# yaomy533/pose_estimation

Hardware: AMD Instinct MI355X
Metric: crops/sec at 640×480 RGB-D, 1000 sampled pts; ADD(-S) AUC vs reference (higher is better)
Workload: dtype f32; 1 GPU; LineMOD 'cat' batch=64/GPU, 120x120 crops from 640x480 RGB-D, HRNet-W18 + 1000-pt fusion + TBase, PnP-RANSAC (H=100) on GPU; batch_per_gpu=64, global_batch=64, crop=120, points=1000, backbone=hrnet_w18, parallelism=single, graph=True, micro_batches=1, pipeline=none, graph_branches=True

## Files before the change

include/krrn_hip.h:

```cpp
#ifndef KRRN_HIP_H
#define KRRN_HIP_H

#include <stdint.h>

#ifdef __cplusplus
extern "C" {
#endif

#define KRRN_OK 0
#define KRRN_EARG (-1)
#define KRRN_ESHAPE (-2)
#define KRRN_EALIGN (-3)
#define KRRN_EUNSUPPORTED (-4)

int krrn_conv2d_f32(const float* in, int in_cs, int in_co, int B, int Hi, int Wi, int cin, int Hg, int Wg,
                    int in_s, int ntaps, const int* tap_dy, const int* tap_dx, const float* wt, int N,
                    int n_store, const float* scale, const float* bias, const float* bias2, int b2_div,
                    const float* res, int res_cs, int res_co, float* out, int out_cs, int out_co, int Ho,
                    int Wo, int osy, int osx, int ooy, int oox, int relu, int out_nchw, int tile, int splits,
                    float* workspace, void* stream);

typedef struct krrn_conv_desc {
  const float* in;
  int in_cs, in_co, B, Hi, Wi, cin, Hg, Wg, in_s, ntaps;
  int tap_dy[9];
  int tap_dx[9];
  const float* wt;
  int N, n_store;
  const float* scale;
  const float* bias;
  const float* bias2;
  int b2_div;
  const float* res;
  int res_cs, res_co;
  float* out;
  int out_cs, out_co, Ho, Wo, osy, osx, ooy, oox, relu, out_nchw, splits;
  float* workspace;
  int k_chunk;
} krrn_conv_desc;

int krrn_conv2d_group_f32(const krrn_conv_desc* descs, int n, int tile, void* stream);

int krrn_conv2d_x3_f32(const float* in, int in_cs, int in_co, int B, int Hi, int Wi, int cin, int Hg, int Wg,
                       int in_s, int ntaps, const int* tap_dy, const int* tap_dx, const void* wt3, int N, int n_store,
                       const float* scale, const float* bias, const float* bias2, int b2_div, const float* res,
                       int res_cs, int res_co, float* out, int out_cs, int out_co, int Ho, int Wo, int osy, int osx,
                       int ooy, int oox, int relu, int tile, int splits, float* workspace, void* stream);
int krrn_conv2d_group_x3_f32(const krrn_conv_desc* descs, int n, int tile, void* stream);
int krrn_convT_s2_x3_f32(const float* in, int in_cs, int in_co, int B, int Hi, int Wi, int cin, const int* cls_taps,
                         const void* U3, int N, const float* scale, const float* bias, int relu, float* out,
                         int out_cs, int out_co, int Ho, int Wo, void* stream);

typedef struct krrn_blas_gemm krrn_blas_gemm;
int krrn_blas_gemm_create(int M, int N, int K, int lda, int ldo, int batch, long long a_grp, long long o_grp,
                          int has_bias, int relu, int has_res, int ldr, long long r_grp, long long max_ws,
                          krrn_blas_gemm** out_plan, long long* ws_bytes);
int krrn_blas_gemm_run(const krrn_blas_gemm* g, const float* a, const float* w, const float* bias, const float* res,
                       float* out, void* workspace, long long ws_bytes, void* stream);
int krrn_blas_gemm_destroy(krrn_blas_gemm* g);

int krrn_gemm_x3_f32(const float* a, int lda, int M, int K, int N, const void* w3f, const float* bias,
                     const float* res, int ldr, float* out, int ldo, int relu, int batch, long long a_grp,
                     long long o_grp, long long r_grp, void* stream);

int krrn_gemm_x3_gather_f32(const int* ia, const float* A, long long a_bs, int a_st, const int* ib, const float* A2,
                            long long a2_bs, int a2_st, int npts, int B, int K, int N, const void* w3f,
                            const float* bias, float* out, int ldo, int relu, void* stream);

int krrn_gemm_panel_x3_f32(const float* a, int lda, int M, int K, int N, const void* wpf, const float* bias,
                           const float* res, int ldr, float* out, int ldo, int relu, int csplit, void* stream);

int krrn_conv1x1_nchw_f32(const float* in, int in_cs, int in_co, int B, int HW, int cin, const float* wt, int N,
                          int n_store, const float* scale, const float* bias, float* out, int out_cs, int out_co,
                          void* stream);

int krrn_conv1x1_nchw_x3_f32(const float* in, int in_cs, int in_co, int B, int HW, int cin, const void* w3, int N,
                             int n_store, const float* scale, const float* bias, float* out, int out_cs, int out_co,
                             void* stream);

int krrn_conv3x3_wino_f32(const float* in, int in_cs, int in_co, int B, int H, int W, int cin, const float* U,
                          int N, int n_store, const float* scale, const float* bias, const float* res, int res_cs,
                          int res_co, float* out, int out_cs, int out_co, int relu, void* stream);
int krrn_conv3x3_wino_x3_f32(const float* in, int in_cs, int in_co, int B, int H, int W, int cin, const void* U3,
                             int N, int n_store, const float* scale, const float* bias, const float* res, int res_cs,
                             int res_co, float* out, int out_cs, int out_co, int relu, void* stream);
int krrn_conv3x3_wino4_x3_f32(const float* in, int in_cs, int in_co, int B, int H, int W, int cin, const void* U3,
                              int N, int n_store, const float* scale, const float* bias, const float* res, int res_cs,
                              int res_co, float* out, int out_cs, int out_co, int relu, void* stream);
int krrn_conv3x3_wino4_x3_head_f32(const float* in, int in_cs, int in_co, int B, int H, int W, int cin,
                                   const void* U3, int N, const float* scale, const float* bias, const float* res,
                                   int res_cs, int res_co, int relu, const float* w1, const float* b1, int p1,
                                   float* part, float* out, int out_c, void* stream);
int krrn_conv3x3_wino_x3_head_f32(const float* in, int in_cs, int in_co, int B, int H, int W, int cin,
                                  const void* U3, int N, const float* scale, const float* bias, const float* res,
                                  int res_cs, int res_co, int relu, const float* w1, const float* b1, int p1,
                                  float* part, float* out, int out_c, void* stream);

int krrn_conv_small_f32(const float* in, int in_cs, int in_co, int B, int H, int W, int cin, const float* wt, int N,
                        int n_store, const float* scale, const float* bias, const float* res, int res_cs, int res_co,
                        float* out, int out_cs, int out_co, int relu, int ksize, int stride, int nw, int ks,
                        void* stream);


int krrn_knn_f32(const float* q, long long q_bs, int q_st, int nq, const int* qidx, const float* c,
                 long long c_bs, int c_st, int nc, int d, int k, int drop_first, int mode, int B, int* out,
                 void* stream);

int krrn_gcn_conv_f32(const int* idx, int n, int k, const float* v, long long v_bs, int v_st, int d,
                      const float* dn, int S, int C, const float* Y, const float* bn_scale, const float* bn_bias,
                      int relu, float* out, long long o_bs, int o_st, int B, void* stream);

int krrn_pool_max_f32(const int* nbr, int nq, int kk, const float* F, long long f_bs, int f_st, int C, float* out,
                      long long o_bs, int o_st, int B, void* stream);

int krrn_resize_bilinear_f32(const float* in, int B, int Hi, int Wi, int in_cs, int in_co, int C, float* out,
                             int Ho, int Wo, int out_cs, int out_co, const float* add, int add_cs, int add_co,
                             int align_corners, int relu, void* stream);

int krrn_add_relu_f32(const float* a, int a_cs, int a_co, const float* b, int b_cs, int b_co, float* out,
                      int o_cs, int o_co, long long npix, int C, int relu, void* stream);

int krrn_nchw_to_nhwc_f32(const float* in, int B, int C, int H, int W, float* out, int o_cs, int o_co,
                          void* stream);

int krrn_heads_select_f32(const float* fx, int Cx, int xyz_off, const float* fn, int Cn, const long long* cls,
                          float* xyz_out, float* nml_out, int B, int H, int W, void* stream);

int krrn_points_gather_f32(const float* cloud, const float* xyz, const float* nml, const long long* choose, int B,
                           int N, int H, int W, float* p9, void* stream);

int krrn_gather_rows_f32(const void* idx, int idx64, long long idx_bs, int nrows, const float* src, long long src_bs,
                         int src_st, float* dst, long long dst_bs, int dst_st, int width, int B, void* stream);

int krrn_gather2_add_f32(const int* ia, const float* A, long long a_bs, int a_st, const int* ib, const float* B_,
                         long long b_bs, int b_st, int n, int C, const float* scale, const float* bias,
                         const float* bias2, int relu, float* out, long long o_bs, int o_st, int B, void* stream);

int krrn_tbase_tail_f32(const float* h, int B, int n, int C, const float* w4, const float* b4, const float* cloud,
                        float* pred_t, float* t_res, void* stream);

int krrn_pnp_ransac_f32(const float* xyz, int HW, const long long* choose, int N, const int* sel, int P,
                        const float* xmap, const float* ymap, const float* K4, const double* extent,
                        const double* lfborder, const int* subsets, int H, float thr, double conf, float* workspace,
                        float* R, float* t, int* inliers, unsigned char* inlier_mask, int B, void* stream);

int krrn_model_points_f32(const float* xyz, int HW, const long long* choose, int N, const double* extent,
                          const double* lfborder, float* out, int B, void* stream);

int krrn_umeyama_ransac_f32(const float* src, const float* dst, int N, const int* subsets, int H,
                            double inlier_frac, double conf, double min_ratio, int* hyp_counts,
                            float* scale, float* R, float* t, int* inliers, int* best_hyp,
                            unsigned char* inlier_mask, int B, void* stream);

int krrn_icp_refine_f32(const float* R0, const float* t0, const float* cloud, int N, const float* model, int M,
                        const float* max_dist, int max_iter, double tol, int min_pairs, float* R, float* t,
                        int* passes, int* pairs, float* rmse, int* status, int* nn_idx, int B, void* stream);

int krrn_randperm_i32(const unsigned long long* seed_ptr, unsigned int stream_id, int n, int k, int rows, int* out,
                      void* stream);

int krrn_randperm_multi_i32(const unsigned long long* seed_ptr, int count, const unsigned int* stream_id, const int* n,
                            const int* k, int* const* out, void* stream);

int krrn_ransac_subsets(const unsigned long long* seed_ptr, unsigned int stream_id, int B, int H, int P, int* out,
                        void* stream);

int krrn_rng_advance(unsigned long long* seed_ptr, void* stream);

int krrn_map_losses_ws(int B, int HW, long long* n_doubles);
int krrn_map_losses_f32(const float* xyz, const float* xyz_gt, const float* nml, const float* nml_gt,
                        const float* region, int R, const long long* region_gt, const float* mask, int M,
                        const long long* mask_gt, int B, int HW, double* ws, double* out, void* stream);
int krrn_map_losses_crop_f32(const double* ws, int B, int HW, double* out_crop, void* stream);

int krrn_pose_loss_ws(int B, int P, long long* n_doubles);
int krrn_pose_loss_f32(const float* target_r, const float* pred_t, const float* target, const float* model_points,
                       const long long* cls_id, const int* sym, int nsym, int B, int P, double* ws, double* out,
                       void* stream);

int krrn_add_metric_f32(const float* pred_r, const float* pred_t, const float* model_points, const float* target,
                        const long long* cls_id, const int* sym, int nsym, int B, int P, double* ws, double* out,
                        void* stream);

int krrn_crop_inputs_u8(const unsigned char* rgb, const float* depth, const unsigned char* mask_label,
                        const unsigned char* obj_mask, int F, int H, int W, const int* frame, const int* rc, int B,
                        int S, float* img, unsigned char* mask, void* stream);

int krrn_choose_points(const unsigned char* mask, int B, int S, int N, const float* depth, int H, int W,
                       const int* frame, const int* rc, const float* K4, float depth_scale, const long long* seed,
                       int stream_id, long long* choose, float* cloud, float* xmap, float* ymap, int* count,
                       void* stream);

int krrn_fps_f32(const float* pts, int B, int n, int n_samples, int* out_idx, void* stream);

int krrn_raster_maps_f32(const float* verts, int Vtot, const int* faces, int Ftot, const int* face_range,
                         const double* R, const double* t, const float* K4, const int* rc, int S,
                         const float* region_pts, int NR, int B, int* face, float* depth, float* coord,
                         float* normal, int* region, unsigned char* cover_frame, int H, int W, void* stream);

int krrn_gt_maps_finish_f32(const float* coord, const int* region_raw, const int* face,
                            const unsigned char* point_mask, const long long* cls, const double* extent,
                            const double* lfborder, int B, int HW, float* xyz, float* normal, long long* region,
                            float* mask, long long* multi_cls_mask, float* mask_obj, void* stream);

int krrn_bop_vsd_ws(int B, long long* n_ints);
int krrn_bop_vsd_f32(const float* verts, int Vtot, const int* faces, int Ftot, const int* face_range,
                     const double* R_est, const double* t_est, const double* R_gt, const double* t_gt,
                     const float* K4, const float* depth, int F, int H, int W, const int* frame, double depth_scale,
                     const double* diameter, double delta, const double* taus, int T, int B, int* ws, int* counts,
                     double* e_vsd, void* stream);

int krrn_bop_visib_ws(int B, long long* n_ints);
int krrn_bop_visib_u8(const float* verts, int Vtot, const int* faces, int Ftot, const int* face_range,
                      const double* R, const double* t, const float* K4, const float* depth, int F, int H, int W,
                      const int* frame, double depth_scale, double delta, int B, int* ws,
                      unsigned char* mask, unsigned char* mask_visib, int* info, double* visib_fract,
                      void* stream);

int krrn_bop_mssd_mspd_ws(int B, long long* n_doubles);
int krrn_bop_mssd_mspd_f32(const float* verts, int Vtot, const int* vert_range, const double* R_est,
                           const double* t_est, const double* R_gt, const double* t_gt, const float* K4,
                           const double* syms, int NStot, const int* sym_range, int B, double* ws, double* mssd,
                           double* mspd, int* sym_idx, void* stream);

int krrn_bpnp_solve_f32(const float* pts2d, const float* pts3d, int z_per_crop, const float* K, const float* y_init,
                        const float* R_init, int B, int n, int iters, float* y_out, float* cost_out, void* stream);

int krrn_bpnp_backward_f32(const float* pts2d, const float* P6, const float* pts3d, int z_per_crop, const float* K,
                           const float* grad_out, int B, int n, float* grad_x, float* grad_z, float* grad_K,
                           double* workspace, void* stream);

#ifdef __cplusplus
}
#endif

#endif
```

pose_estimation_amd/csrc/gemm_x3.hip:

```cpp
#include "krrn_common.h"
#include "krrn_split.h"

namespace {

constexpr int BM = 128, BN = 128;
constexpr int KC = 16;
constexpr int NG = KC / 8;
constexpr int PX = 3 * KC + 4;

struct GemmArgs {
  const float* a;
  const float* a2;
  const int* ia;
  const int* ib;
  long long a2_grp;
  int lda2, npts;
  const unsigned* w;
  const float* bias;
  const float* res;
  float* out;
  int lda, M, K, N, ldr, ldo, relu;
  long long a_grp, o_grp, r_grp;
  int mt, nt, total;
};

__device__ __forceinline__ void split_quads(const f32x4 x, u32x4& q0, u32x4& q1, u32x4& q2) {
  const KrrnSplit3 s = krrn_split3(x);
  q0 = u32x4{s.h0, s.h1, s.h0, s.h1};
  q1 = u32x4{s.h0, s.h1, s.m0, s.m1};
  q2 = u32x4{s.m0, s.m1, s.l0, s.l1};
}

template <bool GA>
__global__ __launch_bounds__(256, 2) void gemm_x3_kernel(const GemmArgs g) {
  __shared__ __attribute__((aligned(16))) unsigned smem[2 * BM * PX];

  const int tpg = g.mt * g.nt;
  const int bid = krrn_xcd_remap(blockIdx.x, g.total);
  const int grp = bid / tpg, rem = bid - grp * tpg;
  const int tm = rem / g.nt, tn = rem - tm * g.nt;
  const int m0 = tm * BM, n0 = tn * BN;
  const int tid = threadIdx.x, lane = tid & 63, wave = tid >> 6;
  const int frow = lane & 31, fh = lane >> 5;

  const int srow = tid >> 2, kq = (tid & 3) * 4;
  const float* abase = GA ? g.a : g.a + grp * g.a_grp + (size_t)m0 * g.lda;
  const int rows = min(BM, g.M - m0);
  const __amdgpu_buffer_rsrc_t rsA = __builtin_amdgcn_make_buffer_rsrc(
      (void*)abase, (short)0, GA ? (int)(g.a_grp * (g.M / g.npts) * 4) : ((rows - 1) * g.lda + g.K) * 4, 0x00020000);
  __amdgpu_buffer_rsrc_t rsA2;
  unsigned aoff[2], aoff2[2];
  if constexpr (GA) {
    rsA2 = __builtin_amdgcn_make_buffer_rsrc((void*)g.a2, (short)0, (int)(g.a2_grp * (g.M / g.npts) * 4),
                                             0x00020000);
#pragma unroll
    for (int i = 0; i < 2; ++i) {
      const int m = m0 + srow + 64 * i;
      if (m < g.M) {
        const int b = m / g.npts;
        aoff[i] = (unsigned)((b * g.a_grp + (long long)g.ia[m] * g.lda + kq) * 4);
        aoff2[i] = (unsigned)((b * g.a2_grp + (long long)g.ib[m] * g.lda2 + kq) * 4);
      } else {
        aoff[i] = aoff2[i] = 0x80000000u;
      }
    }
  } else {
#pragma unroll
    for (int i = 0; i < 2; ++i) aoff[i] = (unsigned)(((srow + 64 * i) * g.lda + kq) * 4);
  }

  const int G = g.K >> 3;
  const unsigned* wb = g.w + ((size_t)((n0 >> 5) + wave) * G) * 512 + lane * 4;

  const int nch = g.K / KC;
  f32x4 ra[2][2];
  f32x4 rq[GA ? 2 : 1][2];
  auto load_a = [&](int c, int s) {
    c = min(c, nch - 1);
#pragma unroll
    for (int i = 0; i < 2; ++i) {
      ra[s][i] = __builtin_bit_cast(
          f32x4, __builtin_amdgcn_raw_buffer_load_b128(rsA, aoff[i] + (unsigned)(c * KC * 4), 0, 0));
      if constexpr (GA)
        rq[s][i] = __builtin_bit_cast(
            f32x4, __builtin_amdgcn_raw_buffer_load_b128(rsA2, aoff2[i] + (unsigned)(c * KC * 4), 0, 0));
    }
  };
  auto store_a = [&](int s) {
    unsigned* d = smem + s * BM * PX;
#pragma unroll
    for (int i = 0; i < 2; ++i) {
      u32x4 q0, q1, q2;
      f32x4 x = ra[s][i];
      if constexpr (GA) {
        x += rq[s][i];
#pragma unroll
        for (int e = 0; e < 4; ++e) x[e] = fmaxf(x[e], 0.f);
      }
      split_quads(x, q0, q1, q2);
      unsigned* p = d + (srow + 64 * i) * PX + 3 * kq;
      *reinterpret_cast<u32x4*>(p) = q0;
      *reinterpret_cast<u32x4*>(p + 4) = q1;
      *reinterpret_cast<u32x4*>(p + 8) = q2;
    }
  };
  u32x4 wr[4][2];
  auto load_w = [&](int gi, int s) {
    const unsigned* p = wb + (size_t)min(gi, G - 1) * 512;
    wr[s][0] = *reinterpret_cast<const u32x4*>(p);
    wr[s][1] = *reinterpret_cast<const u32x4*>(p + 256);
  };

  f32x16 acc[4];
#pragma unroll
  for (int i = 0; i < 4; ++i)
#pragma unroll
    for (int r = 0; r < 16; ++r) acc[i][r] = 0.f;
  typedef u32x4 Frag[4][3];
  auto read_frag = [&](int buf, int gl, Frag& f) {
    const unsigned* As = smem + buf * BM * PX;
#pragma unroll
    for (int i = 0; i < 4; ++i) {
      const unsigned* p = As + (i * 32 + frow) * PX + 12 * (2 * gl + fh);
#pragma unroll
      for (int q = 0; q < 3; ++q) f[i][q] = *reinterpret_cast<const u32x4*>(p + 4 * q);
    }
  };
  auto mma = [&](const Frag& f, int s) {
    const bf16x8 p0 = krrn_op(wr[s][0]), p1 = krrn_op(wr[s][1]);
#pragma unroll
    for (int i = 0; i < 4; ++i) {
      acc[i] = __builtin_amdgcn_mfma_f32_32x32x16_bf16(krrn_op(f[i][0]), p0, acc[i], 0, 0, 0);
      acc[i] = __builtin_amdgcn_mfma_f32_32x32x16_bf16(krrn_op(f[i][1]), p1, acc[i], 0, 0, 0);
      acc[i] = __builtin_amdgcn_mfma_f32_32x32x16_bf16(krrn_op(f[i][2]), p1, acc[i], 0, 0, 0);
    }
  };

  static_assert(NG == 2, "the chunk schedule below is written for 2 groups per chunk");
  Frag fa, fb;
  load_a(0, 0);
  load_a(1, 1);
  load_w(0, 0);
  load_w(1, 1);
  store_a(0);
  __syncthreads();
  load_a(2, 0);
  read_frag(0, 0, fa);
  for (int c = 0; c < nch; c += 2) {
#pragma unroll
    for (int h = 0; h < 2; ++h) {
      const int gi = (c + h) * NG;
      __builtin_amdgcn_sched_barrier(0);
      load_w(gi + 2, (2 * h + 2) & 3);
      read_frag(h, 1, fb);
      store_a(1 - h);
      mma(fa, 2 * h);
      __builtin_amdgcn_sched_group_barrier(0x020, 2, 0);
      __builtin_amdgcn_sched_group_barrier(0x100, 12, 0);
#pragma unroll
      for (int q = 0; q < 12; ++q) {
        __builtin_amdgcn_sched_group_barrier(0x008, 1, 0);
        __builtin_amdgcn_sched_group_barrier(0x002, 6, 0);
        if (q < 6) __builtin_amdgcn_sched_group_barrier(0x200, 1, 0);
      }
      __builtin_amdgcn_sched_barrier(0);
      __syncthreads();
      load_a(c + h + 3, 1 - h);
      load_w(gi + 3, (2 * h + 3) & 3);
      read_frag(1 - h, 0, fa);
      __builtin_amdgcn_sched_barrier(0);
      mma(fb, 2 * h + 1);
    }
  }
  __builtin_amdgcn_sched_barrier(0);

  __syncthreads();
  constexpr int TP = 36;
  float* const ts = reinterpret_cast<float*>(smem) + wave * (32 * TP);
  const int trow = lane >> 3, tcol = 4 * (lane & 7);
  const int nq = n0 + wave * 32 + tcol;
  float bq[4];
#pragma unroll
  for (int e = 0; e < 4; ++e) bq[e] = g.bias ? g.bias[nq + e] : 0.f;
  float* ob = g.out + grp * g.o_grp + nq;
  const float* rb = g.res ? g.res + grp * g.r_grp + nq : nullptr;
#pragma unroll
  for (int i = 0; i < 4; ++i) {
#pragma unroll
    for (int r = 0; r < 16; ++r) ts[((r & 3) + 8 * (r >> 2) + 4 * fh) * TP + frow] = acc[i][r];
    __builtin_amdgcn_wave_barrier();
    f32x4 tv[4];
#pragma unroll
    for (int j = 0; j < 4; ++j) tv[j] = *reinterpret_cast<const f32x4*>(ts + (8 * j + trow) * TP + tcol);
    __builtin_amdgcn_wave_barrier();
#pragma unroll
    for (int j = 0; j < 4; ++j) {
      const int m = m0 + i * 32 + 8 * j + trow;
      if (m >= g.M) continue;
      f32x4 v = tv[j];
#pragma unroll
      for (int e = 0; e < 4; ++e) {
        v[e] += bq[e];
        if (rb) v[e] += rb[(size_t)m * g.ldr + e];
        if (g.relu) v[e] = fmaxf(v[e], 0.f);
      }
      *reinterpret_cast<f32x4*>(ob + (size_t)m * g.ldo) = v;
    }
  }
}

}

KRRN_API int krrn_gemm_x3_f32(const float* a, int lda, int M, int K, int N, const void* w3f, const float* bias,
                              const float* res, int ldr, float* out, int ldo, int relu, int batch, long long a_grp,
                              long long o_grp, long long r_grp, void* stream) {
  if (!a || !w3f || !out) return KRRN_EARG;
  if (M < 1 || K < KC || N < BN || batch < 1) return KRRN_ESHAPE;
  if ((K % (2 * KC)) || (N % BN) || lda < K || ldo < N) return KRRN_ESHAPE;
  if ((lda & 3) || (ldo & 3) || (a_grp & 3) || (o_grp & 3)) return KRRN_EALIGN;
  if (res && ((ldr != 0 && ldr < N) || (r_grp & 3))) return KRRN_ESHAPE;
  if (!krrn_aligned16(a) || !krrn_aligned16(w3f) || !krrn_aligned16(out)) return KRRN_EALIGN;
  if ((long long)BM * lda * 4 >= 0x7FFFFFFFLL) return KRRN_ESHAPE;
  const long long tiles = (long long)krrn_cdiv(M, BM) * (N / BN) * batch;
  if (tiles > 0x7FFFFFFFLL) return KRRN_ESHAPE;
  GemmArgs g;
  g.a = a; g.a2 = nullptr; g.ia = g.ib = nullptr; g.a2_grp = 0; g.lda2 = 0; g.npts = 1;
  g.w = reinterpret_cast<const unsigned*>(w3f); g.bias = bias; g.res = res; g.out = out;
  g.lda = lda; g.M = M; g.K = K; g.N = N; g.ldr = ldr; g.ldo = ldo; g.relu = relu;
  g.a_grp = a_grp; g.o_grp = o_grp; g.r_grp = r_grp;
  g.mt = krrn_cdiv(M, BM); g.nt = N / BN; g.total = (int)tiles;
  hipLaunchKernelGGL(gemm_x3_kernel<false>, dim3((unsigned)tiles), dim3(256), 0, (hipStream_t)stream, g);
  return krrn_launch_status();
}

KRRN_API int krrn_gemm_x3_gather_f32(const int* ia, const float* A, long long a_bs, int a_st, const int* ib,
                                     const float* A2, long long a2_bs, int a2_st, int npts, int B, int K, int N,
                                     const void* w3f, const float* bias, float* out, int ldo, int relu,
                                     void* stream) {
  if (!ia || !A || !ib || !A2 || !w3f || !out) return KRRN_EARG;
  if (npts < 1 || B < 1 || K < KC || N < BN) return KRRN_ESHAPE;
  if ((K % (2 * KC)) || (N % BN) || a_st < K || a2_st < K || ldo < N) return KRRN_ESHAPE;
  if ((a_st & 3) || (a2_st & 3) || (a_bs & 3) || (a2_bs & 3) || (ldo & 3)) return KRRN_EALIGN;
  if (!krrn_aligned16(A) || !krrn_aligned16(A2) || !krrn_aligned16(w3f) || !krrn_aligned16(out)) return KRRN_EALIGN;
  if ((long long)B * a_bs * 4 >= 0x7FFFFFFFLL || (long long)B * a2_bs * 4 >= 0x7FFFFFFFLL) return KRRN_ESHAPE;
  const long long M = (long long)B * npts;
  const long long tiles = (long long)krrn_cdiv(M, BM) * (N / BN);
  if (M > 0x7FFFFFFFLL || tiles > 0x7FFFFFFFLL) return KRRN_ESHAPE;
  GemmArgs g;
  g.a = A; g.a2 = A2; g.ia = ia; g.ib = ib; g.a_grp = a_bs; g.a2_grp = a2_bs; g.lda = a_st; g.lda2 = a2_st;
  g.npts = npts;
  g.w = reinterpret_cast<const unsigned*>(w3f); g.bias = bias; g.res = nullptr; g.out = out;
  g.M = (int)M; g.K = K; g.N = N; g.ldr = 0; g.ldo = ldo; g.relu = relu;
  g.o_grp = 0; g.r_grp = 0;
  g.mt = krrn_cdiv(g.M, BM); g.nt = N / BN; g.total = (int)tiles;
  hipLaunchKernelGGL(gemm_x3_kernel<true>, dim3((unsigned)tiles), dim3(256), 0, (hipStream_t)stream, g);
  return krrn_launch_status();
}
```

pose_estimation_amd/csrc/pointwise.hip:

```cpp
#include <math.h>

#include "krrn_common.h"

namespace {

template <typename IT>
__global__ void resize_bilinear_kernel(const float* __restrict__ in, int Hi, int Wi, int in_cs, int in_co, int C4,
                                       float* __restrict__ out, int Ho, int Wo, int out_cs, int out_co,
                                       const float* __restrict__ add, int add_cs, int add_co, float sh, float sw,
                                       int align, int relu, IT total) {
  const IT e = (IT)blockIdx.x * blockDim.x + threadIdx.x;
  if (e >= total) return;
  const int c4 = (int)(e % C4);
  IT p = e / C4;
  const int ox = (int)(p % Wo);
  p /= Wo;
  const int oy = (int)(p % Ho);
  const int b = (int)(p / Ho);
  int y0, y1, x0, x1;
  float ly0, ly1, lx0, lx1;
  krrn_src_index(oy, Hi, sh, align, y0, y1, ly0, ly1);
  krrn_src_index(ox, Wi, sw, align, x0, x1, lx0, lx1);
  const float* ib = in + (long long)b * Hi * Wi * in_cs + in_co + 4 * c4;
  const f32x4 v00 = *reinterpret_cast<const f32x4*>(ib + ((long long)y0 * Wi + x0) * in_cs);
  const f32x4 v01 = *reinterpret_cast<const f32x4*>(ib + ((long long)y0 * Wi + x1) * in_cs);
  const f32x4 v10 = *reinterpret_cast<const f32x4*>(ib + ((long long)y1 * Wi + x0) * in_cs);
  const f32x4 v11 = *reinterpret_cast<const f32x4*>(ib + ((long long)y1 * Wi + x1) * in_cs);
  f32x4 r = krrn_bilerp4(v00, v01, v10, v11, ly0, ly1, lx0, lx1);
  const long long opix = ((long long)b * Ho + oy) * Wo + ox;
  if (add) r = *reinterpret_cast<const f32x4*>(add + opix * add_cs + add_co + 4 * c4) + r;
  if (relu) {
    r.x = fmaxf(r.x, 0.f); r.y = fmaxf(r.y, 0.f); r.z = fmaxf(r.z, 0.f); r.w = fmaxf(r.w, 0.f);
  }
  *reinterpret_cast<f32x4*>(out + opix * out_cs + out_co + 4 * c4) = r;
}

__device__ __forceinline__ f32x4 pick3(const f32x4 (&r)[3], int i) { return i == 0 ? r[0] : (i == 1 ? r[1] : r[2]); }

__global__ void resize_up2x2_kernel(const float* __restrict__ in, int Hi, int Wi, int in_cs, int in_co, int C4,
                                    float* __restrict__ out, int Ho, int Wo, int out_cs, int out_co,
                                    const float* __restrict__ add, int add_cs, int add_co, float sh, float sw,
                                    int align, int relu, int Ho2, int Wo2, int total) {
  const int e = blockIdx.x * blockDim.x + threadIdx.x;
  if (e >= total) return;
  const int c4 = e % C4;
  int p = e / C4;
  const int ox2 = p % Wo2;
  p /= Wo2;
  const int oy2 = p % Ho2;
  const int b = p / Ho2;
  int y0[2], y1[2], x0[2], x1[2];
  float ly0[2], ly1[2], lx0[2], lx1[2];
#pragma unroll
  for (int d = 0; d < 2; ++d) {
    krrn_src_index(min(2 * oy2 + d, Ho - 1), Hi, sh, align, y0[d], y1[d], ly0[d], ly1[d]);
    krrn_src_index(min(2 * ox2 + d, Wo - 1), Wi, sw, align, x0[d], x1[d], lx0[d], lx1[d]);
  }
  const float* ib = in + (long long)b * Hi * Wi * in_cs + in_co + 4 * c4;
  f32x4 P[3][3];
#pragma unroll
  for (int r = 0; r < 3; ++r)
#pragma unroll
    for (int c = 0; c < 3; ++c) {
      const int yy = min(y0[0] + r, Hi - 1), xx = min(x0[0] + c, Wi - 1);
      P[r][c] = *reinterpret_cast<const f32x4*>(ib + ((long long)yy * Wi + xx) * in_cs);
    }
#pragma unroll
  for (int dy = 0; dy < 2; ++dy) {
    const int oy = 2 * oy2 + dy;
    if (oy >= Ho) break;
    const int ra = y0[dy] - y0[0], rb = y1[dy] - y0[0];
    f32x4 row0[3], row1[3];
#pragma unroll
    for (int c = 0; c < 3; ++c) {
      row0[c] = ra == 0 ? P[0][c] : P[1][c];
      row1[c] = rb == 0 ? P[0][c] : (rb == 1 ? P[1][c] : P[2][c]);
    }
#pragma unroll
    for (int dx = 0; dx < 2; ++dx) {
      const int ox = 2 * ox2 + dx;
      if (ox >= Wo) break;
      const int ca = x0[dx] - x0[0], cb = x1[dx] - x0[0];
      const f32x4 v00 = pick3(row0, ca), v01 = pick3(row0, cb), v10 = pick3(row1, ca), v11 = pick3(row1, cb);
      f32x4 r = krrn_bilerp4(v00, v01, v10, v11, ly0[dy], ly1[dy], lx0[dx], lx1[dx]);
      const long long opix = ((long long)b * Ho + oy) * Wo + ox;
      if (add) r = *reinterpret_cast<const f32x4*>(add + opix * add_cs + add_co + 4 * c4) + r;
      if (relu) {
        r.x = fmaxf(r.x, 0.f); r.y = fmaxf(r.y, 0.f); r.z = fmaxf(r.z, 0.f); r.w = fmaxf(r.w, 0.f);
      }
      *reinterpret_cast<f32x4*>(out + opix * out_cs + out_co + 4 * c4) = r;
    }
  }
}

template <typename IT>
__global__ void add_relu_kernel(const float* __restrict__ a, int a_cs, int a_co, const float* __restrict__ b,
                                int b_cs, int b_co, float* __restrict__ out, int o_cs, int o_co, int C4, int relu,
                                IT total) {
  const IT e = (IT)blockIdx.x * blockDim.x + threadIdx.x;
  if (e >= total) return;
  const int c4 = (int)(e % C4);
  const long long pix = e / C4;
  f32x4 r = *reinterpret_cast<const f32x4*>(a + pix * a_cs + a_co + 4 * c4);
  if (b) r = r + *reinterpret_cast<const f32x4*>(b + pix * b_cs + b_co + 4 * c4);
  if (relu) {
    r.x = fmaxf(r.x, 0.f); r.y = fmaxf(r.y, 0.f); r.z = fmaxf(r.z, 0.f); r.w = fmaxf(r.w, 0.f);
  }
  *reinterpret_cast<f32x4*>(out + pix * o_cs + o_co + 4 * c4) = r;
}

__global__ void nchw_to_nhwc_kernel(const float* __restrict__ in, int C, int HW, float* __restrict__ out, int o_cs,
                                    int o_co, long long total) {
  const long long e = (long long)blockIdx.x * blockDim.x + threadIdx.x;
  if (e >= total) return;
  const int p = (int)(e % HW);
  const long long bc = e / HW;
  const int c = (int)(bc % C);
  const long long b = bc / C;
  out[(b * HW + p) * o_cs + o_co + c] = in[e];
}

__global__ void heads_select_kernel(const float* __restrict__ fx, int Cx, int xyz_off, const float* __restrict__ fn,
                                    int Cn, const long long* __restrict__ cls, float* __restrict__ xyz,
                                    float* __restrict__ nml, int HW, long long total) {
  const long long e = (long long)blockIdx.x * blockDim.x + threadIdx.x;
  if (e >= total) return;
  const int p = (int)(e % HW);
  const long long b = e / HW;
  const int c = (int)cls[b];
  const float* sx = fx + (b * Cx + xyz_off + 3 * c) * HW + p;
  const float* sn = fn + (b * Cn + 3 * c) * HW + p;
  float* dx = xyz + b * 3 * HW + p;
  float* dn = nml + b * 3 * HW + p;
  dx[0] = sx[0];
  dx[HW] = sx[HW];
  dx[2 * HW] = sx[2 * HW];
  const float n0 = sn[0], n1 = sn[HW], n2 = sn[2 * HW];
  const float nr = fmaxf(sqrtf(n0 * n0 + n1 * n1 + n2 * n2), 1e-12f);
  dn[0] = n0 / nr;
  dn[HW] = n1 / nr;
  dn[2 * HW] = n2 / nr;
}

__global__ void points_gather_kernel(const float* __restrict__ cloud, const float* __restrict__ xyz,
                                     const float* __restrict__ nml, const long long* __restrict__ choose, int N,
                                     int HW, float* __restrict__ p9, long long total) {
  const long long e = (long long)blockIdx.x * blockDim.x + threadIdx.x;
  if (e >= total) return;
  const long long b = e / N;
  const long long pix = choose[e];
  float* o = p9 + e * 9;
  const float* cl = cloud + e * 3;
  o[0] = cl[0];
  o[1] = cl[1];
  o[2] = cl[2];
  const float* x = xyz + b * 3 * HW + pix;
  const float* n = nml + b * 3 * HW + pix;
  o[3] = x[0];
  o[4] = x[HW];
  o[5] = x[2 * HW];
  o[6] = n[0];
  o[7] = n[HW];
  o[8] = n[2 * HW];
}

template <bool IDX64, bool VEC>
__global__ void gather_rows_kernel(const void* __restrict__ idx, long long idx_bs, int nrows,
                                   const float* __restrict__ src, long long src_bs, int src_st,
                                   float* __restrict__ dst, long long dst_bs, int dst_st, int width,
                                   long long total) {
  const long long e = (long long)blockIdx.x * blockDim.x + threadIdx.x;
  if (e >= total) return;
  const int wq = VEC ? width / 4 : width;
  const int w = (int)(e % wq);
  const long long br = e / wq;
  const int r = (int)(br % nrows);
  const long long b = br / nrows;
  const long long ii = b * idx_bs + r;
  const long long row = IDX64 ? ((const long long*)idx)[ii] : (long long)((const int*)idx)[ii];
  const float* s = src + b * src_bs + row * src_st;
  float* d = dst + b * dst_bs + (long long)r * dst_st;
  if constexpr (VEC) {
    *reinterpret_cast<f32x4*>(d + 4 * w) = *reinterpret_cast<const f32x4*>(s + 4 * w);
  } else {
    d[w] = s[w];
  }
}

constexpr int kTailWaves = 16;
__global__ __launch_bounds__(64 * kTailWaves) void tbase_tail_kernel(const float* __restrict__ h, int n, int C,
                                                         const float* __restrict__ w4,
                                                         const float* __restrict__ b4,
                                                         const float* __restrict__ cloud,
                                                         float* __restrict__ pred_t, float* __restrict__ t_res) {
  __shared__ float red[kTailWaves][3];
  const int b = blockIdx.x;
  const int lane = threadIdx.x & 63, wave = threadIdx.x >> 6;
  const int q = lane & 3, pl = lane >> 2;
  const int C4 = C >> 2;
  const float bx = b4[0], by = b4[1], bz = b4[2];
  float sx = 0.f, sy = 0.f, sz = 0.f;
  for (int i0 = 0; i0 < n; i0 += 16 * kTailWaves) {
    const int i = i0 + wave * 16 + pl;
    if (i < n) {
      const f32x4* hr = reinterpret_cast<const f32x4*>(h + ((long long)b * n + i) * C);
      float a0 = 0.f, a1 = 0.f, a2 = 0.f;
      for (int c4 = q; c4 < C4; c4 += 4) {
        const f32x4 x = hr[c4];
        const f32x4 w0 = reinterpret_cast<const f32x4*>(w4)[c4];
        const f32x4 w1 = reinterpret_cast<const f32x4*>(w4 + C)[c4];
        const f32x4 w2 = reinterpret_cast<const f32x4*>(w4 + 2 * C)[c4];
        a0 += w0[0] * x[0] + w0[1] * x[1] + w0[2] * x[2] + w0[3] * x[3];
        a1 += w1[0] * x[0] + w1[1] * x[1] + w1[2] * x[2] + w1[3] * x[3];
        a2 += w2[0] * x[0] + w2[1] * x[1] + w2[2] * x[2] + w2[3] * x[3];
      }
      a0 += __shfl_xor(a0, 1);
      a1 += __shfl_xor(a1, 1);
      a2 += __shfl_xor(a2, 1);
      a0 += __shfl_xor(a0, 2);
      a1 += __shfl_xor(a1, 2);
      a2 += __shfl_xor(a2, 2);
      if (q == 0) {
        const float t0 = a0 + bx, t1 = a1 + by, t2 = a2 + bz;
        if (t_res) {
          float* tr = t_res + ((long long)b * n + i) * 3;
          tr[0] = t0; tr[1] = t1; tr[2] = t2;
        }
        const float* cp = cloud + ((long long)b * n + i) * 3;
        sx += cp[0] + t0;
        sy += cp[1] + t1;
        sz += cp[2] + t2;
      }
    }
  }
#pragma unroll
  for (int off = 4; off < 64; off <<= 1) {
    sx += __shfl_xor(sx, off);
    sy += __shfl_xor(sy, off);
    sz += __shfl_xor(sz, off);
  }
  if (lane == 0) {
    red[wave][0] = sx; red[wave][1] = sy; red[wave][2] = sz;
  }
  __syncthreads();
  if (threadIdx.x < 3) {
    const int j = threadIdx.x;
    float acc = 0.f;
#pragma unroll
    for (int w = 0; w < kTailWaves; ++w) acc += red[w][j];
    pred_t[b * 3 + j] = acc / (float)n;
  }
}

template <typename IT>
__global__ void gather2_add_kernel(const int* __restrict__ ia, const float* __restrict__ A, long long a_bs, int a_st,
                                   const int* __restrict__ ib, const float* __restrict__ Bm, long long b_bs,
                                   int b_st, int n, int C4, const float* __restrict__ scale,
                                   const float* __restrict__ bias, const float* __restrict__ bias2, int relu,
                                   float* __restrict__ out, long long o_bs, int o_st, IT total) {
  const IT e = (IT)blockIdx.x * blockDim.x + threadIdx.x;
  if (e >= total) return;
  const int c4 = (int)(e % C4);
  const IT bi = e / C4;
  const int i = (int)(bi % n);
  const int b = (int)(bi / n);
  const int ra = ia[(long long)b * n + i], rb = ib[(long long)b * n + i];
  const f32x4 x = *reinterpret_cast<const f32x4*>(A + b * a_bs + (long long)ra * a_st + 4 * c4) +
                  *reinterpret_cast<const f32x4*>(Bm + b * b_bs + (long long)rb * b_st + 4 * c4);
  f32x4 v = x * *reinterpret_cast<const f32x4*>(scale + 4 * c4) + *reinterpret_cast<const f32x4*>(bias + 4 * c4);
  if (bias2) v += *reinterpret_cast<const f32x4*>(bias2 + (long long)b * 4 * C4 + 4 * c4);
  if (relu) {
    v.x = fmaxf(v.x, 0.f); v.y = fmaxf(v.y, 0.f); v.z = fmaxf(v.z, 0.f); v.w = fmaxf(v.w, 0.f);
  }
  *reinterpret_cast<f32x4*>(out + b * o_bs + (long long)i * o_st + 4 * c4) = v;
}

inline dim3 grid1(long long total) { return dim3((unsigned)((total + 255) / 256)); }

}

KRRN_API int krrn_resize_bilinear_f32(const float* in, int B, int Hi, int Wi, int in_cs, int in_co, int C,
                                      float* out, int Ho, int Wo, int out_cs, int out_co, const float* add,
                                      int add_cs, int add_co, int align_corners, int relu, void* stream) {
  if (!in || !out) return KRRN_EARG;
  if (B < 1 || Hi < 1 || Wi < 1 || Ho < 1 || Wo < 1 || C < 1) return KRRN_ESHAPE;
  if ((C & 3) || (in_cs & 3) || (in_co & 3) || (out_cs & 3) || (out_co & 3) || !krrn_aligned16(in) ||
      !krrn_aligned16(out))
    return KRRN_EALIGN;
  if (add && ((add_cs & 3) || (add_co & 3) || !krrn_aligned16(add))) return KRRN_EALIGN;
  float sh, sw;
  if (align_corners) {
    sh = Ho > 1 ? (float)(Hi - 1) / (float)(Ho - 1) : 0.f;
    sw = Wo > 1 ? (float)(Wi - 1) / (float)(Wo - 1) : 0.f;
  } else {
    sh = (float)Hi / (float)Ho;
    sw = (float)Wi / (float)Wo;
  }
  const int Ho2 = (Ho + 1) / 2, Wo2 = (Wo + 1) / 2;
  const long long total2 = (long long)B * Ho2 * Wo2 * (C / 4);
  constexpr long long up_min = 1LL << 21;
  if (Ho >= Hi && Wo >= Wi && total2 >= up_min && total2 < 0x7fffffffLL) {
    hipLaunchKernelGGL(resize_up2x2_kernel, grid1(total2), dim3(256), 0, (hipStream_t)stream, in, Hi, Wi, in_cs, in_co,
                       C / 4, out, Ho, Wo, out_cs, out_co, add, add_cs, add_co, sh, sw, align_corners, relu, Ho2, Wo2,
                       (int)total2);
    return krrn_launch_status();
  }
  const long long total = (long long)B * Ho * Wo * (C / 4);
  if (total < 0x7fffffffLL)
    hipLaunchKernelGGL(resize_bilinear_kernel<int>, grid1(total), dim3(256), 0, (hipStream_t)stream, in, Hi, Wi,
                       in_cs, in_co, C / 4, out, Ho, Wo, out_cs, out_co, add, add_cs, add_co, sh, sw, align_corners,
                       relu, (int)total);
  else
    hipLaunchKernelGGL(resize_bilinear_kernel<long long>, grid1(total), dim3(256), 0, (hipStream_t)stream, in, Hi,
                       Wi, in_cs, in_co, C / 4, out, Ho, Wo, out_cs, out_co, add, add_cs, add_co, sh, sw,
                       align_corners, relu, total);
  return krrn_launch_status();
}

KRRN_API int krrn_add_relu_f32(const float* a, int a_cs, int a_co, const float* b, int b_cs, int b_co, float* out,
                               int o_cs, int o_co, long long npix, int C, int relu, void* stream) {
  if (!a || !out) return KRRN_EARG;
  if (npix < 1 || C < 1) return KRRN_ESHAPE;
  if ((C & 3) || (a_cs & 3) || (a_co & 3) || (o_cs & 3) || (o_co & 3) || (b && ((b_cs & 3) || (b_co & 3))))
    return KRRN_EALIGN;
  if (!krrn_aligned16(a) || !krrn_aligned16(out) || (b && !krrn_aligned16(b))) return KRRN_EALIGN;
  const long long total = npix * (C / 4);
  if (total < 0x7fffffffLL)
    hipLaunchKernelGGL(add_relu_kernel<int>, grid1(total), dim3(256), 0, (hipStream_t)stream, a, a_cs, a_co, b, b_cs,
                       b_co, out, o_cs, o_co, C / 4, relu, (int)total);
  else
    hipLaunchKernelGGL(add_relu_kernel<long long>, grid1(total), dim3(256), 0, (hipStream_t)stream, a, a_cs, a_co, b,
                       b_cs, b_co, out, o_cs, o_co, C / 4, relu, total);
  return krrn_launch_status();
}

KRRN_API int krrn_nchw_to_nhwc_f32(const float* in, int B, int C, int H, int W, float* out, int o_cs, int o_co,
                                   void* stream) {
  if (!in || !out) return KRRN_EARG;
  if (B < 1 || C < 1 || H < 1 || W < 1 || o_co + C > o_cs) return KRRN_ESHAPE;
  const long long total = (long long)B * C * H * W;
  hipLaunchKernelGGL(nchw_to_nhwc_kernel, grid1(total), dim3(256), 0, (hipStream_t)stream, in, C, H * W, out, o_cs,
                     o_co, total);
  return krrn_launch_status();
}

KRRN_API int krrn_heads_select_f32(const float* fx, int Cx, int xyz_off, const float* fn, int Cn,
                                   const long long* cls, float* xyz_out, float* nml_out, int B, int H, int W,
                                   void* stream) {
  if (!fx || !fn || !cls || !xyz_out || !nml_out) return KRRN_EARG;
  if (B < 1 || H < 1 || W < 1 || Cx < xyz_off + 3 || Cn < 3) return KRRN_ESHAPE;
  const long long total = (long long)B * H * W;
  hipLaunchKernelGGL(heads_select_kernel, grid1(total), dim3(256), 0, (hipStream_t)stream, fx, Cx, xyz_off, fn, Cn,
                     cls, xyz_out, nml_out, H * W, total);
  return krrn_launch_status();
}

KRRN_API int krrn_points_gather_f32(const float* cloud, const float* xyz, const float* nml, const long long* choose,
                                    int B, int N, int H, int W, float* p9, void* stream) {
  if (!cloud || !xyz || !nml || !choose || !p9) return KRRN_EARG;
  if (B < 1 || N < 1 || H < 1 || W < 1) return KRRN_ESHAPE;
  const long long total = (long long)B * N;
  hipLaunchKernelGGL(points_gather_kernel, grid1(total), dim3(256), 0, (hipStream_t)stream, cloud, xyz, nml, choose,
                     N, H * W, p9, total);
  return krrn_launch_status();
}

KRRN_API int krrn_gather_rows_f32(const void* idx, int idx64, long long idx_bs, int nrows, const float* src,
                                  long long src_bs, int src_st, float* dst, long long dst_bs, int dst_st, int width,
                                  int B, void* stream) {
  if (!idx || !src || !dst) return KRRN_EARG;
  if (B < 1 || nrows < 1 || width < 1) return KRRN_ESHAPE;
  const bool vec = !(width & 3) && !(src_st & 3) && !(dst_st & 3) && !(src_bs & 3) && !(dst_bs & 3) &&
                   krrn_aligned16(src) && krrn_aligned16(dst);
  const long long total = (long long)B * nrows * (vec ? width / 4 : width);
  hipStream_t s = (hipStream_t)stream;
#define KRRN_GR(I64, V)                                                                                    \
  hipLaunchKernelGGL((gather_rows_kernel<I64, V>), grid1(total), dim3(256), 0, s, idx, idx_bs, nrows, src, \
                     src_bs, src_st, dst, dst_bs, dst_st, width, total)
  if (idx64) {
    if (vec) KRRN_GR(true, true); else KRRN_GR(true, false);
  } else {
    if (vec) KRRN_GR(false, true); else KRRN_GR(false, false);
  }
#undef KRRN_GR
  return krrn_launch_status();
}

KRRN_API int krrn_tbase_tail_f32(const float* h, int B, int n, int C, const float* w4, const float* b4,
                                 const float* cloud, float* pred_t, float* t_res, void* stream) {
  if (!h || !w4 || !b4 || !cloud || !pred_t) return KRRN_EARG;
  if (B < 1 || n < 1 || C < 1) return KRRN_ESHAPE;
  if ((C & 3) || !krrn_aligned16(h) || !krrn_aligned16(w4)) return KRRN_EALIGN;
  hipLaunchKernelGGL(tbase_tail_kernel, dim3(B), dim3(64 * kTailWaves), 0, (hipStream_t)stream, h, n, C, w4, b4, cloud, pred_t,
                     t_res);
  return krrn_launch_status();
}

KRRN_API int krrn_gather2_add_f32(const int* ia, const float* A, long long a_bs, int a_st, const int* ib, const float* B_,
                                  long long b_bs, int b_st, int n, int C, const float* scale, const float* bias,
                                  const float* bias2, int relu, float* out, long long o_bs, int o_st, int B,
                                  void* stream) {
  if (!ia || !A || !ib || !B_ || !scale || !bias || !out) return KRRN_EARG;
  if (n < 1 || C < 1 || B < 1) return KRRN_ESHAPE;
  if ((C & 3) || (a_st & 3) || (b_st & 3) || (o_st & 3) || (a_bs & 3) || (b_bs & 3) || (o_bs & 3) ||
      !krrn_aligned16(A) || !krrn_aligned16(B_) || !krrn_aligned16(out) || !krrn_aligned16(scale) ||
      !krrn_aligned16(bias) || (bias2 && !krrn_aligned16(bias2)))
    return KRRN_EALIGN;
  const long long total = (long long)B * n * (C / 4);
  if (total < 0x7fffffffLL)
    hipLaunchKernelGGL(gather2_add_kernel<int>, grid1(total), dim3(256), 0, (hipStream_t)stream, ia, A, a_bs, a_st, ib,
                       B_, b_bs, b_st, n, C / 4, scale, bias, bias2, relu, out, o_bs, o_st, (int)total);
  else
    hipLaunchKernelGGL(gather2_add_kernel<long long>, grid1(total), dim3(256), 0, (hipStream_t)stream, ia, A, a_bs,
                       a_st, ib, B_, b_bs, b_st, n, C / 4, scale, bias, bias2, relu, out, o_bs, o_st, total);
  return krrn_launch_status();
}
```

pose_estimation_amd/fusion.py:

```python
from __future__ import annotations

import math
from typing import Callable, Dict, List, Optional

import torch
import torch.nn as nn
import torch.nn.functional as F

from . import knobs, ops
from .runtime import Late, Plan, add_conv, add_gemm, ptr


class Conv_surface(nn.Module):
    def __init__(self, kernel_num, support_num):
        super().__init__()
        self.kernel_num = kernel_num
        self.support_num = support_num
        self.directions = nn.Parameter(torch.empty(3, support_num * kernel_num))
        stdv = 1.0 / math.sqrt(support_num * kernel_num)
        nn.init.uniform_(self.directions, -stdv, stdv)


class Conv_layer(nn.Module):
    dim = 3

    def __init__(self, in_channel, out_channel, support_num):
        super().__init__()
        self.in_channel, self.out_channel, self.support_num = in_channel, out_channel, support_num
        self.weights = nn.Parameter(torch.empty(in_channel, (support_num + 1) * out_channel))
        self.bias = nn.Parameter(torch.empty((support_num + 1) * out_channel))
        self.directions = nn.Parameter(torch.empty(self.dim, support_num * out_channel))
        stdv = 1.0 / math.sqrt(out_channel * (support_num + 1))
        for p in (self.weights, self.bias, self.directions):
            nn.init.uniform_(p, -stdv, stdv)


class Conv_fuse_layer(Conv_layer):
    dim = 9


class Pool_layer(nn.Module):
    def __init__(self, pooling_rate: int = 4, neighbor_num: int = 4):
        super().__init__()
        self.pooling_rate = pooling_rate
        self.neighbor_num = neighbor_num


class FusionNetLite(nn.Module):
    def __init__(self, cfg):
        super().__init__()
        self.neighbor_num = cfg.Module.GCN3D.GCN_N_NUM
        self.support_num = cfg.Module.GCN3D.GCN_SUP_NUM
        self.num_cls = cfg.Module.NUM_CLS
        S = self.support_num
        for br in ("v", "x", "n"):
            setattr(self, f"conv_0_{br}", Conv_surface(128, S))
            setattr(self, f"conv_1_{br}", Conv_layer(128, 128, S))
            setattr(self, f"pool_1_{br}", Pool_layer(4, 4))
            setattr(self, f"conv_2_{br}", Conv_layer(128, 128, S))
            setattr(self, f"bn1_{br}", nn.BatchNorm1d(128))
            setattr(self, f"bn2_{br}", nn.BatchNorm1d(128))
        self.pool_1 = Pool_layer(4, 4)
        self.pool_2 = Pool_layer(4, 4)
        self.conv_4 = Conv_fuse_layer(384, 512, S)
        self.conv_5 = Conv_fuse_layer(512, 512, S)



FEAT_SID = 4
FUSION_CHUNK = knobs.integer("KRRN_FUSION_CHUNK")

def level_sizes(N: int, k0: int):
    N1 = int(N / 4)
    N2 = int(N1 / 4)
    k1 = min(k0, N1 // 8)
    k2 = min(k0, N2 // 8)
    return N1, N2, k1, k2


def _dn(directions: torch.Tensor, device) -> torch.Tensor:
    return F.normalize(directions.detach().float().cpu(), dim=0).contiguous().to(device)


def _bn1d(bn: nn.BatchNorm1d, device):
    s = (bn.weight.detach().double() / torch.sqrt(bn.running_var.detach().double() + bn.eps))
    b = bn.bias.detach().double() - bn.running_mean.detach().double() * s
    return s.float().to(device), b.float().to(device)


class _Emit:

    def __init__(self, fu: FusionNetLite, plan: Plan, B: int, keep: list):
        self.plan, self.B, self.dev, self.S, self.keep = plan, B, plan.device, fu.support_num, keep
        self._lin: dict = {}

    def knn(self, q, q_bs, q_st, nq, qidx, c, c_bs, c_st, nc, d, k, drop, mode, out):
        self.plan.add("krrn_knn_f32", q, q_bs, q_st, nq, qidx, c, c_bs, c_st, nc, d, k, drop, mode, self.B, ptr(out))

    def gcn(self, idx, n, k, v, v_bs, d, dn, C, Y, bn, relu, out, o_bs, o_st, Bc=None, v_st=9):
        self.keep.append(dn)
        s, b = (None, None) if bn is None else bn
        self.keep.extend([s, b])
        self.plan.add("krrn_gcn_conv_f32", ptr(idx), n, k, v, v_bs, v_st, d, ptr(dn), self.S, C, ptr(Y), ptr(s), ptr(b),
                      int(relu), out, o_bs, o_st, self.B if Bc is None else Bc)

    def gemm(self, a, a_cs, a_co, M, layer: "Conv_layer", out):
        spec = self._lin.get(id(layer))
        if spec is None:
            spec = ops.make_linear(layer.weights.detach().t(), layer.bias, None, self.dev,
                                   cin_p=ops.pad4(layer.in_channel))
            self._lin[id(layer)] = spec
            self.keep.append(spec)
        np_ = ops.pad4(spec.cout)
        if add_gemm(self.plan, a=a, a_off=a_co, lda=a_cs, M=M, wt=spec.wt[0], K=spec.cin_p, N=np_, scale=spec.scale,
                    bias=spec.bias, out=out, ldo=out.shape[-1], relu=False, cin=spec.cin, cout=spec.cout,
                    tag="gcn_gemm"):
            return
        add_conv(self.plan, x=ptr(a), x_cs=a_cs, x_co=a_co, B=1, Hi=1, Wi=M, cin_p=spec.cin_p, Hg=1, Wg=M, in_s=1,
                 taps=[(0, 0)], wt=ptr(spec.wt[0]), N=np_, n_store=np_, scale=ptr(spec.scale), bias=ptr(spec.bias),
                 out=ptr(out), out_cs=out.shape[-1], out_co=0, Ho=1, Wo=M, cin=spec.cin, cout=spec.cout,
                 tag="gcn_gemm")


def _off(t, floats):
    return ptr(t) if floats == 0 else type(ptr(t))(t.data_ptr() + 4 * floats)


def _level0_branch(e: _Emit, fu: FusionNetLite, bi: int, br: str, N: int, idx0, v, v_bs, v_st, F0, Y1b, feat1, cy: int):
    B = e.B
    c0 = getattr(fu, f"conv_0_{br}")
    e.gcn(idx0, N, fu.neighbor_num, v, v_bs, 3, _dn(c0.directions, e.dev), 128, None, None, True,
          _off(F0, 128 * bi), N * 384, 384, v_st=v_st)
    c1 = getattr(fu, f"conv_1_{br}")
    dn1, bn1 = _dn(c1.directions, e.dev), _bn1d(getattr(fu, f"bn1_{br}"), e.dev)
    for b0 in range(0, B, cy):
        nb = min(cy, B - b0)
        e.gemm(F0[b0:b0 + nb], 384, 128 * bi, nb * N, c1, Y1b)
        vb = type(v)(v.value + 4 * b0 * v_bs)
        e.gcn(idx0[b0:b0 + nb], N, fu.neighbor_num, vb, v_bs, 3, dn1, 128, Y1b, bn1, True,
              _off(feat1[b0:], 128 * bi), N * 384, 384, Bc=nb, v_st=v_st)


def emit_fusion_cloud_part(fu: FusionNetLite, plan: Plan, B: int, N: int, cloud: torch.Tensor) -> dict:
    k0 = fu.neighbor_num
    keep: list = []
    e = _Emit(fu, plan, B, keep)
    cy = B if not FUSION_CHUNK or FUSION_CHUNK >= B else FUSION_CHUNK
    idx0 = plan.buf((B, N, k0), torch.int32)
    F0 = plan.buf((B, N, 384))
    feat1 = plan.buf((B, N, 384))
    Y1v = plan.buf((cy * N, (fu.support_num + 1) * 128))
    e.knn(ptr(cloud), N * 3, 3, N, ptr(None), ptr(cloud), N * 3, 3, N, 3, k0, 1, 0, idx0)
    _level0_branch(e, fu, 0, "v", N, idx0, ptr(cloud), N * 3, 3, F0, Y1v, feat1, cy)
    plan.buffers.append(keep)
    return dict(idx0=idx0, F0=F0, feat1=feat1, Y1v=Y1v)


def build_fusion_plan(fu: FusionNetLite, plan: Plan, B: int, N: int, p9: torch.Tensor, perms: Dict[str, torch.Tensor],
                      hooks: Optional[Dict[str, List[Callable[[dict], None]]]] = None, materialize: bool = True,
                      early: Optional[dict] = None):
    hooks = hooks or {}
    dev = plan.device
    S = fu.support_num
    k0 = fu.neighbor_num
    N1, N2, k1, k2 = level_sizes(N, k0)
    if k1 < 1 or k2 < 1:
        raise ValueError(f"num_points={N} too small for the 3-level GCN (needs N/16 >= 8)")
    keep = []
    i32 = torch.int32
    idx0 = early["idx0"] if early else plan.buf((B, N, k0), i32)
    F0 = early["F0"] if early else plan.buf((B, N, 384))
    cy = B if not FUSION_CHUNK or FUSION_CHUNK >= B else FUSION_CHUNK
    Y1 = [early["Y1v"] if early and i == 0 else plan.buf((cy * N, (S + 1) * 128)) for i in range(3)]
    feat1 = early["feat1"] if early else plan.buf((B, N, 384))
    nb4 = {br: plan.buf((B, N1, 4), i32) for br in ("v", "x", "n")}
    V1 = plan.buf((B, N1, 9))
    FP1 = plan.buf((B, N1, 384))
    PV1 = plan.buf((B, N1, 9))
    idx1 = plan.buf((B, N1, k1), i32)
    Y2 = [plan.buf((B * N1, (S + 1) * 128)) for _ in range(3)]
    feat2 = plan.buf((B, N1, 384))
    nb4b = plan.buf((B, N2, 4), i32)
    FP2 = plan.buf((B, N2, 384))
    PV2 = plan.buf((B, N2, 9))
    idx2 = plan.buf((B, N2, k2), i32)
    Y4 = plan.buf((B * N2, (S + 1) * 512))
    fm4 = plan.buf((B, N2, 512))
    Y5 = plan.buf((B * N2, (S + 1) * 512))
    fm5 = plan.buf((B, N2, 512))
    nn1 = plan.buf((B, N), i32)
    nn2 = plan.buf((B, N), i32)
    feat = plan.buf((B, N, 1280)) if materialize else None

    e = _Emit(fu, plan, B, keep)
    knn, gcn, gemm, off = e.knn, e.gcn, e.gemm, _off

    if not early:
        knn(off(p9, 0), N * 9, 9, N, ptr(None), off(p9, 0), N * 9, 9, N, 3, k0, 1, 0, idx0)
    plan.fork([1, 2])
    for bi, br in enumerate(("v", "x", "n")):
        with plan.on_stream(bi):
            if not (early and bi == 0):
                _level0_branch(e, fu, bi, br, N, idx0, off(p9, 3 * bi), N * 9, 9, F0, Y1[bi], feat1, cy)
            perm = perms[br]
            knn(off(p9, 3 * bi), N * 9, 9, N1, ptr(perm), off(p9, 3 * bi), N * 9, 9, N, 3, 4, 1, 0, nb4[br])
            plan.add("krrn_pool_max_f32", ptr(nb4[br]), N1, 4, off(feat1, 128 * bi), N * 384, 384, 128,
                     off(FP1, 128 * bi), N1 * 384, 384, B)
            plan.add("krrn_gather_rows_f32", ptr(perm), 0, 0, N1, off(p9, 3 * bi), N * 9, 9, off(V1, 3 * bi),
                     N1 * 9, 9, 3, B)
    plan.add("krrn_gather_rows_f32", ptr(perms["p1"]), 0, 0, N1, off(p9, 0), N * 9, 9, off(PV1, 0), N1 * 9, 9, 9, B)
    plan.join([1, 2])
    knn(off(V1, 0), N1 * 9, 9, N1, ptr(None), off(V1, 0), N1 * 9, 9, N1, 3, k1, 1, 0, idx1)
    plan.fork([1, 2, 3])
    with plan.on_stream(3):
        knn(off(p9, 0), N * 9, 9, N, ptr(None), off(PV1, 0), N1 * 9, 9, N1, 3, 1, 0, 1, nn1)
    for bi, br in enumerate(("v", "x", "n")):
        with plan.on_stream(bi):
            c2 = getattr(fu, f"conv_2_{br}")
            gemm(FP1, 384, 128 * bi, B * N1, c2, Y2[bi])
            gcn(idx1, N1, k1, off(V1, 3 * bi), N1 * 9, 3, _dn(c2.directions, dev), 128, Y2[bi],
                _bn1d(getattr(fu, f"bn2_{br}"), dev), True, off(feat2, 128 * bi), N1 * 384, 384)
    plan.join([1, 2])
    for h in hooks.get("level1", []):
        h(dict(feat1=feat1, feat2=feat2))
    knn(off(PV1, 0), N1 * 9, 9, N2, ptr(perms["p2"]), off(PV1, 0), N1 * 9, 9, N1, 3, 4, 1, 0, nb4b)
    plan.add("krrn_pool_max_f32", ptr(nb4b), N2, 4, off(feat2, 0), N1 * 384, 384, 384, off(FP2, 0), N2 * 384, 384, B)
    plan.add("krrn_gather_rows_f32", ptr(perms["p2"]), 0, 0, N2, off(PV1, 0), N1 * 9, 9, off(PV2, 0), N2 * 9, 9, 9, B)
    knn(off(PV2, 0), N2 * 9, 9, N2, ptr(None), off(PV2, 0), N2 * 9, 9, N2, 9, k2, 1, 0, idx2)
    for h in hooks.get("level2", []):
        h(dict(feat1=feat1, feat2=feat2))
    plan.fork([3])
    with plan.on_stream(3):
        knn(off(p9, 0), N * 9, 9, N, ptr(None), off(PV2, 0), N2 * 9, 9, N2, 3, 1, 0, 1, nn2)
    gemm(FP2, 384, 0, B * N2, fu.conv_4, Y4)
    gcn(idx2, N2, k2, off(PV2, 0), N2 * 9, 9, _dn(fu.conv_4.directions, dev), 512, Y4, None, False,
        off(fm4, 0), N2 * 512, 512)
    gemm(fm4, 512, 0, B * N2, fu.conv_5, Y5)
    gcn(idx2, N2, k2, off(PV2, 0), N2 * 9, 9, _dn(fu.conv_5.directions, dev), 512, Y5, None, False,
        off(fm5, 0), N2 * 512, 512)
    plan.join([3])
    if materialize:
        plan.fork([FEAT_SID])
        with plan.on_stream(FEAT_SID):
            plan.add("krrn_gather_rows_f32", ptr(nn2), 0, N, N, off(fm5, 0), N2 * 512, 512, off(feat, 0), N * 1280,
                     1280, 512, B)
            plan.add("krrn_gather_rows_f32", ptr(nn1), 0, N, N, off(feat1, 0), N * 384, 384, off(feat, 512),
                     N * 1280, 1280, 384, B)
            plan.add("krrn_gather_rows_f32", ptr(nn1), 0, N, N, off(feat2, 0), N1 * 384, 384, off(feat, 896),
                     N * 1280, 1280, 384, B)
    plan.buffers.append(keep)
    return feat, dict(pool_v=nb4["v"], pool_x=nb4["x"], pool_n=nb4["n"], pool2=nb4b, idx0=idx0, idx1=idx1, idx2=idx2, nn1=nn1, nn2=nn2, feat1=feat1, feat2=feat2, fm5=fm5,
                      F0=F0, V1=V1, PV1=PV1, PV2=PV2, FP1=FP1, FP2=FP2, fm4=fm4, Y1=Y1, Y2=Y2, Y4=Y4, Y5=Y5)
```

pose_estimation_amd/knobs.py:

```python
from __future__ import annotations

import os
from typing import Dict, Optional, Tuple

KNOBS: Dict[str, Tuple[Optional[str], str]] = {
    "KRRN_HIP_LIB": (None, "path of the C-ABI library to load instead of the in-tree libkrrn_hip.so "
                           "(variant builds for A/B timing, the KRRN_DIAG diagnostics build)"),
    "KRRN_GRAPH": ("1", "KRRN.forward replays a captured hipGraph of its plan; 0 = serial eager runs"),
    "KRRN_PLAN_STREAMS": ("1", "captured plans keep their side streams as graph branches; 0 = captured serially"),
    "KRRN_STREAMS": ("1", "the two-slot pipeline's stages, concurrent micro-batches and config 3's buckets "
                          "replay side by side on their own streams; 0 = one after the other"),
    "KRRN_PLAN_BUDGET_GB": ("48", "device memory the KRRN plan cache may hold before evicting the least "
                                  "recently used (B, S, N) plan"),
    "KRRN_DIAG_DROP": ("", "comma list of C-ABI entry points left out of new plans: a what-if timing "
                           "diagnostic (profiles/whatif.sh); outputs are meaningless with it set"),
    "KRRN_WINO": ("1", "3x3 stride-1 convs on the Winograd kernels; 0 = the implicit-GEMM conv"),
    "KRRN_WINO_X3": ("1", "Winograd with split-bf16 MFMAs (f32 accuracy); 0 = the f32 Winograd"),
    "KRRN_WINO4": ("1", "the heads' wide 3x3 convs on the split-bf16 Winograd F(4x4, 3x3); 0 = F(2x2, 3x3)"),
    "KRRN_FUSE_EARLY": ("1", "HRNet fuse terms that read one branch start on that branch's stream before the join"),
    "KRRN_MODULE_STREAMS": ("1", "consecutive HRNet modules of a stage keep each branch on its stream (no barrier between them)"),
    "KRRN_STAGE_STREAMS": ("1", "with KRRN_MODULE_STREAMS, HRNet stages chain per branch stream too (transitions on their branch's stream)"),
    "KRRN_FUSION_EARLY": ("1", "the fusion work that reads only the input cloud runs beside the HRNet phase (side stream)"),
    "KRRN_FUSE_EDGES": ("1", "each HRNet fuse output waits for exactly its branches (capture edges); 0 = module barrier"),
    "KRRN_HEAD_FUSE": ("1", "a <= 4-output final 1x1 fused into the head's last split Winograd; 0 = two launches"),
    "KRRN_SMALL_CONV": ("1", "HRNet branch / fuse convs on the LDS-slab conv_small kernel; 0 = implicit GEMM"),
    "KRRN_GEMM_1X1": ("1", "stride-1 1x1 convs as plain GEMMs; 0 = implicit-GEMM conv"),
    "KRRN_CONVT_S2": ("1", "stride-2 transposed convs with 128 outputs on the all-classes-per-block kernel (convt.hip); 0 = the grouped implicit GEMM"),
    "KRRN_DECONV_FOLD": ("1", "fold last_layer_2 into the deconv (272 instead of 400 input channels); "
                              "0 = the literal cat + deconv"),
    "KRRN_FUSE_ID_FIRST": ("1", "HRNet fuse sums start from the identity branch; 0 = the reference's j order"),
    "KRRN_BLAS": ("1", "GEMMs no hand-written kernel takes go to hipBLASLt; 0 = the implicit-GEMM conv"),
    "KRRN_GEMM_X3": ("1", "GEMMs with K >= 256 on the split-bf16 GEMM"),
    "KRRN_GEMM_PANEL": ("1", "K = 64 / 128 GEMMs on the A-stationary panel GEMM"),
    "KRRN_SPLITK": ("1", "split-K for implicit-GEMM convs with few output tiles; 0 = never"),
    "KRRN_TBASE_EARLY": ("1", "TBase conv1's level-1 half runs as soon as level 1 is done (side stream)"),
    "KRRN_TBASE_GATHER": ("1", "TBase conv1 / conv2 by linearity on the fusion's level rows (gathered "
                               "GEMM); 0 = on the materialised 1280-wide concat"),
    "KRRN_POSE_AT": ("level1", "where the fused pose step forks off the forward plan: level1 / level2 / heads"),
    "KRRN_FUSION_CHUNK": ("16", "crops per chunk of the level-0 GCN GEMM + gather-conv, through a chunk-sized "
                                "Y buffer per branch (0 = the whole batch at once; same results)"),
}


def text(name: str) -> Optional[str]:
    if name not in KNOBS:
        raise KeyError(f"{name} is not a declared knob (pose_estimation_amd/knobs.py)")
    return os.environ.get(name, KNOBS[name][0])


def flag(name: str) -> bool:
    return text(name) == "1"


def integer(name: str) -> int:
    return int(text(name))
```

pose_estimation_amd/krrn.py:

```python
from __future__ import annotations

import ctypes
from collections import OrderedDict

from typing import Dict, List, Optional, Sequence, Tuple

import torch
import torch.nn as nn

from . import knobs, ops
from .config import CONFIG
from .fusion import FEAT_SID, FusionNetLite, build_fusion_plan, emit_fusion_cloud_part, level_sizes
from .hrnet import _Builder, build_hrnet, build_hrnet_plan
from .ops import Act, pad4
from .posenet import PoseNet, build_tbase_plan, emit_tbase_level1
from .runtime import Late, Plan, RngStream, add_conv, h2d, ptr



TBASE_EARLY = knobs.flag("KRRN_TBASE_EARLY")
GRAPH = knobs.flag("KRRN_GRAPH")
FUSION_EARLY = knobs.flag("KRRN_FUSION_EARLY")


class KRRNPlan:

    POSE_SID = 6
    TBASE_SID = 5
    CLOUD_SID = 7
    POSE_AT = knobs.text("KRRN_POSE_AT")

    def __init__(self, model: "KRRN", B: int, S: int, N: int, opt_pose: bool, device, pose_hook=None,
                 pose_stream: bool = True):
        with torch.random.fork_rng(devices=[]):
            self._build(model, B, S, N, opt_pose, device, pose_hook, pose_stream)

    def _build(self, model: "KRRN", B: int, S: int, N: int, opt_pose: bool, device, pose_hook, pose_stream):
        self.B, self.S, self.N, self.opt_pose = B, S, N, opt_pose
        cfg = model.cfg
        C = model.num_cls
        plan = Plan(device)
        self.plan = plan
        self.x_in = plan.buf((B, 3, S, S))
        self.cloud = plan.buf((B, N, 3))
        self.choose = plan.buf((B, 1, N), torch.int64)
        self.cls = plan.buf((B, 1), torch.int64)
        self.seed = torch.zeros(1, dtype=torch.int64, device=device)
        xa = Act(plan.buf((B, S, S, 4)), B, S, S, 4, 0, 3)
        plan.add("krrn_nchw_to_nhwc_f32", ptr(self.x_in), B, 3, S, S, ptr(xa.t), 4, 0)
        fe = {}

        def emit_cloud_part():
            plan.fork([self.CLOUD_SID])
            e0 = len(plan.ops)
            with plan.on_stream(self.CLOUD_SID):
                fe["early"] = emit_fusion_cloud_part(model.fusion, plan, B, N, self.cloud)
            fe["ids"] = {id(op) for op in plan.ops[e0:] if op.name != "sync"}

        xmap, ymap, specs = build_hrnet_plan(model.backbone, plan, xa,
                                             after_layer1=emit_cloud_part if FUSION_EARLY and opt_pose else None)
        early, early_ids = fe.get("early"), fe.get("ids", set())
        if early is not None:
            plan.join([self.CLOUD_SID])
        self.split = len(plan.ops)
        self.backbone_out = (xmap.t, ymap.t)
        bld = _Builder(plan, B)
        plan.fork([1])
        X = model.XYZNet
        h = bld.conv(xmap, X[0], X[1], relu=True)
        h = bld.conv(h, X[3], X[4], relu=True)
        self.xyz_outc = model.xyz_outc
        Ho, Wo = 2 * h.H, 2 * h.W
        self.fx = plan.buf((B, model.xyz_outc, Ho, Wo))
        self._head_tail(bld, h, [(X[7], X[8]), (X[10], X[11])], model.xyz_final, self.fx, model.xyz_outc)
        Nn = model.NMLNet
        with plan.on_stream(1):
            g = bld.conv(ymap, Nn[0], Nn[1], relu=True)
            g = bld.conv(g, Nn[3], Nn[4], relu=True)
            self.fn = plan.buf((B, 3 * C, Ho, Wo))
            self._head_tail(bld, g, [(Nn[7], Nn[8])], model.nml_final, self.fn, 3 * C)
        plan.join([1])
        self.Ho, self.Wo = Ho, Wo
        self.xyz = plan.buf((B, 3, Ho, Wo))
        self.normal = plan.buf((B, 3, Ho, Wo))
        plan.add("krrn_heads_select_f32", ptr(self.fx), model.xyz_outc, model.region_outc, ptr(self.fn), 3 * C,
                 ptr(self.cls), ptr(self.xyz), ptr(self.normal), B, Ho, Wo)
        self.heads_end = len(plan.ops)
        self.specs = [specs, bld.specs]
        self.pred_t = None
        psid = self.POSE_SID if pose_stream else 0

        def emit_pose():
            plan.fork([psid])
            with plan.on_stream(psid):
                pose_hook(self)

        pose_at = self.POSE_AT if (pose_hook is not None and opt_pose) else "heads"
        if pose_hook is not None and pose_at == "heads":
            emit_pose()
        if opt_pose:
            self.p9 = plan.buf((B, N, 9))
            plan.add("krrn_points_gather_f32", ptr(self.cloud), ptr(self.xyz), ptr(self.normal), ptr(self.choose), B, N,
                     Ho, Wo, ptr(self.p9))
            N1, N2, _, _ = level_sizes(N, model.fusion.neighbor_num)
            self.perm_sizes = [("v", N, N1), ("x", N, N1), ("n", N, N1), ("p1", N, N1), ("p2", N1, N2)]
            self.perms = {k: plan.buf((m,), torch.int32) for k, _, m in self.perm_sizes}
            self.perm_ops_start = len(plan)
            self.device_perm_plan = Plan(device)
            cnt = len(self.perm_sizes)
            sids = (ctypes.c_uint * cnt)(*RngStream.POOL)
            ns = (ctypes.c_int * cnt)(*[n for _, n, _ in self.perm_sizes])
            ms = (ctypes.c_int * cnt)(*[m for _, _, m in self.perm_sizes])
            outs = (ctypes.c_void_p * cnt)(*[self.perms[k].data_ptr() for k, _, _ in self.perm_sizes])
            self.device_perm_plan.add("krrn_randperm_multi_i32", ptr(self.seed), cnt, sids, ns, ms, outs)
            hooks = {"level1": [], "level2": []}
            side_ids = set()

            def tracked(fn):
                def run(fb):
                    n0 = len(plan.ops)
                    fn(fb)
                    side_ids.update(id(op) for op in plan.ops[n0:])
                return run

            if pose_hook is not None and pose_at != "heads":
                hooks[pose_at].append(tracked(lambda fb: emit_pose()))
            tb_pre = {}
            tb_sid = self.TBASE_SID if pose_stream else 0

            def emit_tb_l1(fb):
                plan.fork([tb_sid])
                with plan.on_stream(tb_sid):
                    tb_pre.update(emit_tbase_level1(model.pose.t_net, plan, B, N, N1, fb["feat1"], fb["feat2"],
                                                      cls_key="cls", inc_r=cfg.Module.POSENet.INC_R, num_cls=C))

            if TBASE_EARLY:
                hooks["level1"].append(tracked(emit_tb_l1))
            f0 = len(plan.ops)
            feat, self.fusion_bufs = build_fusion_plan(model.fusion, plan, B, N, self.p9, self.perms, hooks=hooks,
                                                       materialize=model.keep_fusion_feat, early=early)
            self.fusion_op_ids = {id(op) for op in plan.ops[f0:] if id(op) not in side_ids and op.name != "sync"}
            self.fusion_op_ids |= early_ids
            self.feat = feat
            fb = self.fusion_bufs
            levels = dict(fm5=fb["fm5"], feat1=fb["feat1"], feat2=fb["feat2"], nn1=fb["nn1"], nn2=fb["nn2"], N1=N1,
                          N2=N2)
            self.pred_t, self.tbase_bufs = build_tbase_plan(model.pose.t_net, plan, B, N, feat, "cls", "cloud",
                                                            cfg.Module.POSENet.INC_R, C, levels=levels,
                                                            pre=tb_pre or None, pre_sid=tb_sid)
            if feat is not None:
                plan.join([FEAT_SID])
        if pose_hook is not None:
            plan.join([psid])
        self.env = {"cls": self.cls, "cloud": self.cloud}
        self.graph: Optional[torch.cuda.CUDAGraph] = None
        self.warm = False
        self.nbytes = plan_bytes(plan) + plan_bytes(getattr(self, "device_perm_plan", None))

    def _head_tail(self, bld: _Builder, x: Act, convs, final: nn.Conv2d, out: torch.Tensor, n_store: int):
        spec = ops.make_conv(final, None, self.plan.device, cin_p=pad4(convs[-1][0].out_channels))
        bld.specs.append(spec)
        h = bld.upsample2(x)
        for i, (conv, bn) in enumerate(convs):
            if i == len(convs) - 1 and bld.conv_head(h, conv, bn, final, out, n_store):
                return
            h = bld.conv(h, conv, bn, relu=True)
        self._nchw_conv(h, spec, out, n_store)

    def _nchw_conv(self, x: Act, spec, out: torch.Tensor, n_store: int):
        B, Cx, Ho, Wo = out.shape
        np_ = pad4(spec.cout)
        if len(spec.taps[0]) == 1 and spec.stride == 1 and spec.cin_p <= 256 and np_ <= 80:
            name, wt = "krrn_conv1x1_nchw_f32", spec.wt[0]
            if spec.cin_p == 128 and np_ > 48:
                name, wt = "krrn_conv1x1_nchw_x3_f32", ops.quad_weights_x3(spec.wt[0], np_, 128)
                self.plan.buffers.append(wt)
            self.plan.add(name, ptr(x.t), x.cs, x.co, x.B, Ho * Wo, spec.cin_p, ptr(wt), np_,
                          n_store, ptr(spec.scale), ptr(spec.bias), ptr(out), Cx, 0,
                          meta=dict(kernel="conv1x1_nchw", flops=2.0 * spec.cin * n_store * B * Ho * Wo,
                                    tag="head_final", M=B * Ho * Wo, N=np_, K=spec.cin_p, splits=1,
                                    mfma_flops=2.0 * spec.cin_p * 16 * ((np_ + 15) // 16) * B * Ho * Wo))
            return
        add_conv(self.plan, x=ptr(x.t), x_cs=x.cs, x_co=x.co, B=x.B, Hi=x.H, Wi=x.W, cin_p=spec.cin_p, Hg=Ho, Wg=Wo,
                 in_s=spec.stride, taps=spec.taps[0], wt=ptr(spec.wt[0]), N=pad4(spec.cout), n_store=n_store,
                 scale=ptr(spec.scale), bias=ptr(spec.bias), out=ptr(out), out_cs=Cx, out_co=0, Ho=Ho, Wo=Wo,
                 nchw=True, cin=spec.cin, cout=n_store, tag="head_final")

    def load_inputs(self, x, p_emb, choose, cls):
        self.x_in.copy_(x, non_blocking=True)
        if self.opt_pose:
            self.cloud.copy_(p_emb, non_blocking=True)
            self.choose.copy_(choose.reshape(self.B, 1, self.N), non_blocking=True)
        self.cls.copy_(cls.reshape(self.B, 1), non_blocking=True)

    def set_perms(self, perms: Optional[Sequence[torch.Tensor]], mode: str):
        if not self.opt_pose:
            return
        if perms is not None:
            for (k, n, m), p in zip(self.perm_sizes, perms):
                self.perms[k].copy_(p.reshape(-1)[:m].to(torch.int32), non_blocking=True)
        elif mode == "host":
            for k, n, m in self.perm_sizes:
                self.perms[k].copy_(h2d(torch.randperm(n)[:m].to(torch.int32), self.perms[k].device), non_blocking=True)
        elif mode == "device":
            self.device_perm_plan.run({})
        else:
            raise ValueError(f"perm_mode {mode!r}")

    def run(self):
        if not GRAPH:
            self.plan.run(self.env)
            return
        if self.graph is not None:
            self.graph.replay()
            return
        if not self.warm:
            self.plan.run(self.env)
            self.warm = True
            return
        cur = torch.cuda.current_stream(self.plan.device)
        cur.synchronize()
        before = torch.cuda.memory_reserved(self.plan.device)
        g = torch.cuda.CUDAGraph()
        with torch.cuda.graph(g):
            self.plan.run(self.env, serial=False)
        self.graph = g
        self.nbytes += max(0, torch.cuda.memory_reserved(self.plan.device) - before)
        g.replay()

    def outputs(self, model: "KRRN") -> Dict[str, Optional[torch.Tensor]]:
        C = model.num_cls
        return {
            "xyz": self.xyz,
            "region": self.fx[:, model.mask_outc:model.region_outc],
            "mask": self.fx[:, 0:model.mask_outc],
            "normal": self.normal,
            "pred_r": None,
            "pred_t": self.pred_t if self.opt_pose else None,
        }


def plan_bytes(plan) -> int:
    if plan is None:
        return 0
    seen, total = set(), 0
    stack = list(plan.buffers)
    visited = set()
    while stack:
        x = stack.pop()
        if id(x) in visited:
            continue
        visited.add(id(x))
        if isinstance(x, torch.Tensor):
            if x.is_cuda:
                st = x.untyped_storage()
                if st.data_ptr() not in seen:
                    seen.add(st.data_ptr())
                    total += st.nbytes()
        elif isinstance(x, (list, tuple)):
            stack.extend(x)
        elif isinstance(x, dict):
            stack.extend(x.values())
        elif hasattr(x, "__dict__") and not isinstance(x, type):
            stack.extend(v for v in vars(x).values() if isinstance(v, (torch.Tensor, list, tuple, dict)))
    return total


PLAN_BUDGET = int(float(knobs.text("KRRN_PLAN_BUDGET_GB")) * (1 << 30))


class KRRN(nn.Module):
    def __init__(self, num_cls: int = 1, cfg=CONFIG):
        super().__init__()
        self.cfg = cfg
        self.num_cls = cfg.Module.NUM_CLS
        self.backbone = build_hrnet(cfg)
        xyz_channels = cfg.Module.XYZNet.HEADEN_FS
        mask_out = cfg.Module.MASKNet.OUT_FS * self.num_cls + 1
        xyz_out = cfg.Module.XYZNet.OUT_FS * self.num_cls
        region_out = cfg.Module.REGIONNet.OUT_FS
        self.mask_outc = mask_out
        self.region_outc = mask_out + region_out
        self.xyz_outc = mask_out + xyz_out + region_out
        nml_channels = cfg.Module.NMLNet.HEADEN_FS
        nml_out = cfg.Module.NMLNet.OUT_FS * self.num_cls
        Cb = cfg.Module.BACKBONE_OUTC
        bn = lambda c: nn.BatchNorm2d(c, eps=1e-05, momentum=0.1, affine=True, track_running_stats=True)
        self.XYZNet = nn.Sequential(
            nn.ConvTranspose2d(Cb, xyz_channels, kernel_size=(3, 3), stride=(2, 2), padding=(1, 1),
                               output_padding=(1, 1), bias=False),
            bn(xyz_channels), nn.ReLU(inplace=True),
            nn.Conv2d(xyz_channels, xyz_channels, (3, 3), (1, 1), (1, 1), bias=False), bn(xyz_channels),
            nn.ReLU(inplace=True),
            nn.UpsamplingBilinear2d(scale_factor=2.0),
            nn.Conv2d(xyz_channels, xyz_channels, (3, 3), (1, 1), (1, 1), bias=False), bn(xyz_channels),
            nn.ReLU(inplace=True),
            nn.Conv2d(xyz_channels, xyz_channels, (3, 3), (1, 1), (1, 1), bias=False), bn(xyz_channels),
            nn.ReLU(inplace=True))
        self.xyz_final = nn.Conv2d(xyz_channels, self.xyz_outc, kernel_size=(1, 1))
        self.NMLNet = nn.Sequential(
            nn.Conv2d(Cb, nml_channels, (3, 3), (1, 1), (1, 1), bias=False), bn(nml_channels), nn.ReLU(inplace=True),
            nn.Conv2d(nml_channels, nml_channels, (3, 3), (1, 1), (1, 1), bias=False), bn(nml_channels),
            nn.ReLU(inplace=True),
            nn.UpsamplingBilinear2d(scale_factor=2.0),
            nn.Conv2d(nml_channels, nml_channels, (3, 3), (1, 1), (1, 1), bias=False), bn(nml_channels),
            nn.ReLU(inplace=True))
        self.nml_final = nn.Conv2d(nml_channels, nml_out, kernel_size=(1, 1))
        self.fusion = FusionNetLite(cfg)
        self.pose = PoseNet(cfg)
        self._plans: "OrderedDict[Tuple, KRRNPlan]" = OrderedDict()
        self.plan_budget_bytes = PLAN_BUDGET
        self.return_views = False
        self.keep_fusion_feat = False
        self.perm_mode = "host"

    def invalidate_plans(self):
        self._plans.clear()

    def load_state_dict(self, state_dict, strict: bool = True, assign: bool = False):
        self.invalidate_plans()
        return super().load_state_dict(state_dict, strict=strict, assign=assign)

    def _apply(self, fn, *args, **kwargs):
        self.invalidate_plans()
        return super()._apply(fn, *args, **kwargs)

    def get_plan(self, B: int, S: int, N: int, opt_pose: bool = True) -> KRRNPlan:
        key = (B, S, N, bool(opt_pose))
        p = self._plans.get(key)
        if p is not None:
            self._plans.move_to_end(key)
            return p
        dev = next(self.parameters()).device
        if dev.type != "cuda":
            raise RuntimeError("KRRN runs on the MI355X HIP path only: call .cuda() first")
        while self._plans and self.plans_bytes() + self._estimate(B, S, N) > self.plan_budget_bytes:
            self._plans.popitem(last=False)
        with torch.no_grad():
            p = KRRNPlan(self, B, S, N, opt_pose, dev)
        self._plans[key] = p
        while len(self._plans) > 1 and self.plans_bytes() > self.plan_budget_bytes:
            self._plans.popitem(last=False)
        return p

    def plans_bytes(self) -> int:
        return sum(p.nbytes for p in self._plans.values())

    def _estimate(self, B: int, S: int, N: int) -> int:
        best = None
        for (b, s, n, _), p in self._plans.items():
            r = (B * S * S) / max(1, b * s * s)
            est = int(p.nbytes * r)
            best = est if best is None else max(best, est)
        return best or 0

    @torch.no_grad()
    def forward(self, x, p_emb, choose, cls, region_point=None, opt_pose=True, perms=None):
        B, _, S, S2 = x.shape
        if S != S2:
            raise ValueError("KRRN crops are square (batchdataset.py:890-961)")
        N = p_emb.shape[1] if opt_pose else 1
        p = self.get_plan(B, S, N, opt_pose)
        p.load_inputs(x, p_emb, choose, cls)
        p.set_perms(perms, self.perm_mode)
        p.run()
        out = p.outputs(self)
        if self.return_views:
            return out
        return {k: (v.clone() if v is not None else None) for k, v in out.items()}
```

pose_estimation_amd/posenet.py:

```python
from __future__ import annotations

from typing import Optional

import torch
import torch.nn as nn

from . import knobs, ops
from .runtime import Late, Plan, add_conv, add_gemm, ptr


TBASE_GATHER = knobs.flag("KRRN_TBASE_GATHER")


class TBase(nn.Module):
    def __init__(self, cfg):
        super().__init__()
        self.f = cfg.Module.POSENet.INC_R + cfg.Module.NUM_CLS
        self.k = cfg.Module.POSENet.OUT_T
        self.conv1 = nn.Conv1d(self.f, 1024, 1)
        self.conv2 = nn.Conv1d(1024, 256, 1)
        self.conv3 = nn.Conv1d(256, 256, 1)
        self.conv4 = nn.Conv1d(256, self.k, 1)
        self.drop1 = nn.Dropout(0.2)
        self.bn1 = nn.BatchNorm1d(1024)
        self.bn2 = nn.BatchNorm1d(256)
        self.bn3 = nn.BatchNorm1d(256)


class PoseNet(nn.Module):
    def __init__(self, cfg):
        super().__init__()
        self.t_net = TBase(cfg)


def _conv1_fold(tb: TBase, inc_r: int, num_cls: int, dev):
    w1 = tb.conv1.weight.detach()[:, :, 0]
    spec1 = ops.make_linear(w1[:, :inc_r], tb.conv1.bias, tb.bn1, dev)
    np1 = ops.pad4(1024)
    colv = torch.zeros(num_cls, np1, device=dev)
    colv[:, :1024] = (spec1.scale[:1024, None] * w1[:, inc_r:inc_r + num_cls].to(dev).float()).t()
    return w1, spec1, colv


def emit_tbase_level1(tb: TBase, plan: Plan, B: int, N: int, N1: int, feat1: torch.Tensor,
                      feat2: torch.Tensor, cls_key: str = "cls", inc_r: int = 1280, num_cls: int = 1) -> dict:
    dev = plan.device
    np1 = ops.pad4(1024)
    if TBASE_GATHER:
        w1, spec1, colv = _conv1_fold(tb, inc_r, num_cls, dev)
        wb = ops.make_linear(w1[:, 512:896], None, None, dev)
        wc = ops.make_linear(w1[:, 896:1280], None, None, dev)
        b2 = plan.buf((B, np1))
        plan.add("krrn_gather_rows_f32", Late(cls_key), 1, 1, 1, ptr(colv), 0, np1, ptr(b2), np1, np1, np1, B)
        Q = plan.buf((B * N1, np1))
        P1 = plan.buf((B * N1, np1))
        ok = add_gemm(plan, a=feat2, a_off=0, lda=384, M=N1, wt=wc.wt[0], K=wc.cin_p, N=np1, scale=spec1.scale,
                      bias=spec1.bias, out=Q, ldo=np1, relu=False, res=b2, ldr=0, batch=B, a_grp=N1 * 384,
                      o_grp=N1 * np1, r_grp=np1, cin=wc.cin, cout=wc.cout, tag="tbase_gemm", require_x3=True) and \
            add_gemm(plan, a=feat1, a_off=0, lda=384, M=N1, wt=wb.wt[0], K=wb.cin_p, N=np1, scale=spec1.scale,
                     bias=None, out=P1, ldo=np1, relu=False, res=Q, ldr=np1, batch=B, a_grp=N * 384,
                     o_grp=N1 * np1, r_grp=N1 * np1, cin=wb.cin, cout=wb.cout, tag="tbase_gemm", require_x3=True)
        if not ok:
            raise RuntimeError("TBase gathered conv2 needs the split-bf16 GEMM (KRRN_GEMM_X3=1)")
        plan.buffers.append([wb, wc, spec1, colv])
        return dict(P1=P1, Q=Q, b2=b2, folded=True)
    w1 = tb.conv1.weight.detach()[:, :, 0]
    wb = ops.make_linear(w1[:, 512:896], None, None, dev)
    wc = ops.make_linear(w1[:, 896:1280], None, None, dev)
    Q = plan.buf((B * N1, np1))
    P1 = plan.buf((B * N1, np1))
    if add_gemm(plan, a=feat2, a_off=0, lda=384, M=B * N1, wt=wc.wt[0], K=wc.cin_p, N=np1, scale=wc.scale,
                bias=wc.bias, out=Q, ldo=np1, relu=False, cin=wc.cin, cout=wc.cout, tag="tbase_gemm") and \
            add_gemm(plan, a=feat1, a_off=0, lda=384, M=N1, wt=wb.wt[0], K=wb.cin_p, N=np1, scale=wb.scale,
                     bias=wb.bias, out=P1, ldo=np1, relu=False, res=Q, ldr=np1, batch=B, a_grp=N * 384,
                     o_grp=N1 * np1, r_grp=N1 * np1, cin=wb.cin, cout=wb.cout, tag="tbase_gemm"):
        plan.buffers.append([wb, wc])
        return dict(P1=P1, Q=Q)
    add_conv(plan, x=ptr(feat2), x_cs=384, x_co=0, B=1, Hi=1, Wi=B * N1, cin_p=wc.cin_p, Hg=1, Wg=B * N1, in_s=1,
             taps=[(0, 0)], wt=ptr(wc.wt[0]), N=np1, n_store=np1, scale=ptr(wc.scale), bias=ptr(wc.bias),
             out=ptr(Q), out_cs=np1, out_co=0, Ho=1, Wo=B * N1, relu=False, cin=wc.cin, cout=wc.cout,
             tag="tbase_gemm")
    add_conv(plan, x=ptr(feat1), x_cs=384, x_co=0, B=B, Hi=1, Wi=N, cin_p=wb.cin_p, Hg=1, Wg=N1,
             in_s=1, taps=[(0, 0)], wt=ptr(wb.wt[0]), N=np1, n_store=np1, scale=ptr(wb.scale), bias=ptr(wb.bias),
             res=ptr(Q), res_cs=np1, res_co=0, out=ptr(P1), out_cs=np1, out_co=0, Ho=1, Wo=N1, relu=False,
             cin=wb.cin, cout=wb.cout, tag="tbase_gemm")
    plan.buffers.append([wb, wc])
    return dict(P1=P1, Q=Q)


def build_tbase_plan(tb: TBase, plan: Plan, B: int, N: int, feat: torch.Tensor, cls_key: str, cloud_key: str,
                     inc_r: int, num_cls: int, levels=None, pre: Optional[dict] = None, pre_sid: int = 0):
    dev = plan.device
    w1, spec1, colv = _conv1_fold(tb, inc_r, num_cls, dev)
    np1 = ops.pad4(1024)
    spec2 = ops.make_linear(tb.conv2.weight, tb.conv2.bias, tb.bn2, dev)
    spec3 = ops.make_linear(tb.conv3.weight, tb.conv3.bias, tb.bn3, dev)
    w4 = tb.conv4.weight.detach()[:3, :, 0].float().contiguous().to(dev)
    b4 = tb.conv4.bias.detach()[:3].float().contiguous().to(dev)
    gathered = levels is not None and TBASE_GATHER
    h1 = None if gathered else plan.buf((B * N, 1024))
    h2 = plan.buf((B * N, 256))
    h3 = plan.buf((B * N, 256))
    pred_t = plan.buf((B, 3))
    M = B * N
    keep = [spec1, spec2, spec3, colv, w4, b4]
    if not gathered:
        b2 = plan.buf((B, np1))
        plan.add("krrn_gather_rows_f32", Late(cls_key), 1, 1, 1, ptr(colv), 0, np1, ptr(b2), np1, np1, np1, B)

    def gemm(a, K, spec, out, bias2=None, rows=M, relu=True):
        np_ = ops.pad4(spec.cout)
        if bias2 is None and add_gemm(plan, a=a, a_off=0, lda=K, M=rows, wt=spec.wt[0], K=spec.cin_p, N=np_,
                                      scale=spec.scale, bias=spec.bias, out=out, ldo=out.shape[-1], relu=relu,
                                      cin=spec.cin, cout=spec.cout, tag="tbase_gemm"):
            return
        add_conv(plan, x=ptr(a), x_cs=K, x_co=0, B=1, Hi=1, Wi=rows, cin_p=spec.cin_p, Hg=1, Wg=rows, in_s=1,
                 taps=[(0, 0)], wt=ptr(spec.wt[0]), N=np_, n_store=np_, scale=ptr(spec.scale), bias=ptr(spec.bias),
                 bias2=ptr(bias2) if bias2 is not None else None, b2_div=N, out=ptr(out), out_cs=out.shape[-1],
                 out_co=0, Ho=1, Wo=rows, relu=relu, cin=spec.cin, cout=spec.cout, tag="tbase_gemm")

    if levels is None:
        gemm(feat, inc_r, spec1, h1, bias2=b2)
    else:
        N1, N2 = levels["N1"], levels["N2"]
        wa = ops.make_linear(w1[:, 0:512], None, None, dev)
        keep += [wa]
        P2 = plan.buf((B * N2, np1))
        if gathered:
            if not add_gemm(plan, a=levels["fm5"], a_off=0, lda=512, M=B * N2, wt=wa.wt[0], K=wa.cin_p, N=np1,
                            scale=spec1.scale, bias=None, out=P2, ldo=np1, relu=False, cin=wa.cin, cout=wa.cout,
                            tag="tbase_gemm", require_x3=True):
                raise RuntimeError("TBase gathered conv2 needs the split-bf16 GEMM (KRRN_GEMM_X3=1)")
        else:
            gemm(levels["fm5"], 512, wa, P2, rows=B * N2, relu=False)
        if pre is None:
            pre = emit_tbase_level1(tb, plan, B, N, N1, levels["feat1"], levels["feat2"], cls_key=cls_key,
                                    inc_r=inc_r, num_cls=num_cls)
        else:
            plan.join([pre_sid])
        P1 = pre["P1"]
        if gathered:
            w2 = tb.conv2.weight.detach()[:, :, 0].to(dev).float() * spec2.scale[:256].reshape(256, 1)
            w3 = ops.gemm_weights_x3(w2.contiguous())
            keep += [w3]
            plan.add("krrn_gemm_x3_gather_f32", ptr(levels["nn1"]), ptr(P1), N1 * np1, np1, ptr(levels["nn2"]),
                     ptr(P2), N2 * np1, np1, N, B, 1024, 256, ptr(w3), ptr(spec2.bias), ptr(h2), 256, 1,
                     meta=dict(kernel="gemm_x3", flops=2.0 * 1024 * 256 * M, tag="tbase_gemm", M=M, N=256, K=1024,
                               splits=1, mfma_flops=2.0 * M * 256 * 1024 * 6 / 16,
                               mfma_bf16_flops=2.0 * M * 256 * 1024 * 6))
        else:
            plan.add("krrn_gather2_add_f32", ptr(levels["nn2"]), ptr(P2), N2 * np1, np1, ptr(levels["nn1"]),
                     ptr(P1), N1 * np1, np1, N, np1, ptr(spec1.scale), ptr(spec1.bias), ptr(b2), 1, ptr(h1),
                     N * 1024, 1024, B)
    if not gathered:
        gemm(h1, 1024, spec2, h2)
    gemm(h2, 256, spec3, h3)
    plan.add("krrn_tbase_tail_f32", ptr(h3), B, N, 256, ptr(w4), ptr(b4), Late(cloud_key), ptr(pred_t), ptr(None))
    plan.buffers.append(keep)
    return pred_t, dict(h1=h1, h2=h2, h3=h3)
```

pose_estimation_amd/runtime.py:

```python
from __future__ import annotations

import ctypes
from contextlib import contextmanager
from typing import Any, Callable, Dict, List, Optional, Sequence, Tuple

import torch

from . import _lib, knobs, ops
from ._lib import P, ptr, stream_ptr

I = ctypes.c_int


class ConvDesc(ctypes.Structure):
    _fields_ = [("in_", P), ("in_cs", I), ("in_co", I), ("B", I), ("Hi", I), ("Wi", I), ("cin", I), ("Hg", I),
                ("Wg", I), ("in_s", I), ("ntaps", I), ("tap_dy", I * 9), ("tap_dx", I * 9), ("wt", P), ("N", I),
                ("n_store", I), ("scale", P), ("bias", P), ("bias2", P), ("b2_div", I), ("res", P), ("res_cs", I),
                ("res_co", I), ("out", P), ("out_cs", I), ("out_co", I), ("Ho", I), ("Wo", I), ("osy", I),
                ("osx", I), ("ooy", I), ("oox", I), ("relu", I), ("out_nchw", I), ("splits", I), ("workspace", P),
                ("k_chunk", I)]

STREAM = "__stream__"


def _skey(sid: int) -> str:
    return STREAM if sid == 0 else f"__stream{sid}__"


def h2d(t: torch.Tensor, device, dtype=None) -> torch.Tensor:
    device = torch.device(device)
    if dtype is not None and t.dtype != dtype and t.device.type == "cpu":
        t = t.to(dtype)
    if t.device.type == "cpu" and device.type == "cuda":
        t = t.contiguous().pin_memory()
    return t.to(device=device, dtype=dtype if dtype is not None else t.dtype, non_blocking=True).contiguous()


class Late:
    __slots__ = ("key",)

    def __init__(self, key: str):
        self.key = key


class Op:
    __slots__ = ("name", "fn", "args", "patches", "meta", "sid")

    def __init__(self, name: str, args: Sequence[Any], meta: Optional[dict] = None, sid: int = 0):
        self.name = name
        self.fn = getattr(_lib.lib(), name)
        self.args = list(args)
        self.patches: List[Tuple[int, str]] = [(i, a.key) for i, a in enumerate(self.args) if isinstance(a, Late)]
        self.meta = meta or {}
        self.sid = sid

    def __call__(self, env: Dict[str, Any]):
        args = self.args
        for i, key in self.patches:
            v = env[key]
            args[i] = P(v.data_ptr()) if isinstance(v, torch.Tensor) else v
        st = self.fn(*args)
        if st != 0:
            _lib.check(st, self.name)


class Sync:
    __slots__ = ("src", "dst", "event", "name", "meta", "sid")

    def __init__(self, src: int, dst: int):
        self.src, self.dst = src, dst
        self.event = torch.cuda.Event() if torch.cuda.is_available() else None
        self.name, self.meta, self.sid = "sync", {}, dst

    def __call__(self, env: Dict[str, Any]):
        streams = env["__streams__"]
        if streams is None:
            return
        self.event.record(streams[self.src])
        streams[self.dst].wait_event(self.event)


class _CaptureDeps:
    _hip = None

    @classmethod
    def hip(cls):
        if cls._hip is None:
            h = ctypes.CDLL("libamdhip64.so")
            h.hipStreamGetCaptureInfo_v2.argtypes = [P, ctypes.POINTER(ctypes.c_int), ctypes.POINTER(ctypes.c_ulonglong),
                                                     ctypes.POINTER(P), ctypes.POINTER(ctypes.POINTER(P)),
                                                     ctypes.POINTER(ctypes.c_size_t)]
            h.hipStreamUpdateCaptureDependencies.argtypes = [P, ctypes.POINTER(P), ctypes.c_size_t, ctypes.c_uint]
            cls._hip = h
        return cls._hip

    @classmethod
    def add(cls, src: "torch.cuda.Stream", dst: "torch.cuda.Stream") -> bool:
        h = cls.hip()
        st, cid, graph = ctypes.c_int(), ctypes.c_ulonglong(), P()
        deps, n = ctypes.POINTER(P)(), ctypes.c_size_t()
        e = h.hipStreamGetCaptureInfo_v2(P(src.cuda_stream), ctypes.byref(st), ctypes.byref(cid), ctypes.byref(graph),
                                         ctypes.byref(deps), ctypes.byref(n))
        if e != 0 or st.value != 1:
            return False
        nodes = (P * max(1, n.value))(*[deps[k] for k in range(n.value)])
        e = h.hipStreamUpdateCaptureDependencies(P(dst.cuda_stream), nodes, n.value, 0)
        if e != 0:
            raise RuntimeError(f"hipStreamUpdateCaptureDependencies failed ({e})")
        return True


class Edge(Sync):
    __slots__ = ()

    def __call__(self, env: Dict[str, Any]):
        streams = env["__streams__"]
        if streams is None:
            return
        if not _CaptureDeps.add(streams[self.src], streams[self.dst]):
            Sync.__call__(self, env)


_DIAG_DROP = frozenset(filter(None, knobs.text("KRRN_DIAG_DROP").split(",")))
PLAN_STREAMS = knobs.flag("KRRN_PLAN_STREAMS")
STREAMS = knobs.flag("KRRN_STREAMS")


class Plan:

    def __init__(self, device: torch.device):
        self.device = device
        self.ops: List[Any] = []
        self.buffers: List[torch.Tensor] = []
        self.cur = 0
        self.nstreams = 1
        self._side: List[torch.cuda.Stream] = []
        self._scratch: Dict[Tuple[int, int], torch.Tensor] = {}
        self._packed: Dict[tuple, torch.Tensor] = {}

    def buf(self, shape, dtype=torch.float32, zero: bool = True) -> torch.Tensor:
        t = (torch.zeros if zero else torch.empty)(tuple(shape), dtype=dtype, device=self.device)
        self.buffers.append(t)
        return t

    def scratch(self, nfloats: int, slot: int = 0) -> torch.Tensor:
        key = (self.cur, slot)
        ws = self._scratch.get(key)
        if ws is None or ws.numel() < nfloats:
            ws = self.buf((max(nfloats, 1 << 20),), zero=False)
            self._scratch[key] = ws
        return ws

    def add(self, name: str, *args, meta: Optional[dict] = None):
        if _DIAG_DROP and name in _DIAG_DROP:
            return
        self.ops.append(Op(name, list(args) + [Late(_skey(self.cur))], meta, self.cur))

    @contextmanager
    def on_stream(self, sid: int):
        prev, self.cur = self.cur, sid
        self.nstreams = max(self.nstreams, sid + 1)
        try:
            yield
        finally:
            self.cur = prev

    def fork(self, sids: Sequence[int]):
        for s in sids:
            if s != 0:
                self.ops.append(Sync(0, s))

    def join(self, sids: Sequence[int]):
        for s in sids:
            if s != 0:
                self.ops.append(Sync(s, 0))

    def sync(self, src: int, dst: int):
        if src != dst:
            self.nstreams = max(self.nstreams, src + 1, dst + 1)
            self.ops.append(Sync(src, dst))

    def edge(self, src: int, dst: int):
        if src != dst:
            self.nstreams = max(self.nstreams, src + 1, dst + 1)
            self.ops.append(Edge(src, dst))

    def side_streams(self) -> List[torch.cuda.Stream]:
        while len(self._side) < self.nstreams - 1:
            self._side.append(torch.cuda.Stream(self.device))
        return self._side

    def _streams(self, env: Dict[str, Any], serial: bool):
        main = torch.cuda.current_stream(self.device)
        self.side_streams()
        streams = [main] + self._side
        for sid in range(self.nstreams):
            env[_skey(sid)] = P((main if serial else streams[sid]).cuda_stream)
        env["__streams__"] = None if serial else streams
        return main

    def run(self, env: Dict[str, Any], serial: bool = True):
        serial = serial or not PLAN_STREAMS
        self._streams(env, serial)
        for op in self.ops:
            op(env)

    def __len__(self):
        return len(self.ops)

    def kernels(self) -> List[Op]:
        return [op for op in self.ops if isinstance(op, Op)]

    def run_timed(self, env: Dict[str, Any]) -> List[Tuple[Op, float]]:
        stream = self._streams(env, serial=True)
        kops = self.kernels()
        evs = [torch.cuda.Event(enable_timing=True) for _ in range(len(kops) + 1)]
        evs[0].record(stream)
        for i, op in enumerate(kops):
            op(env)
            evs[i + 1].record(stream)
        stream.synchronize()
        return [(op, evs[i].elapsed_time(evs[i + 1])) for i, op in enumerate(kops)]


class Immediate:

    def __init__(self, device):
        self.device = torch.device(device)

    def buf(self, shape, dtype=torch.float32) -> torch.Tensor:
        return torch.empty(tuple(shape), dtype=dtype, device=self.device)

    def add(self, name: str, *args):
        _lib.call(name, *args, stream_ptr(self.device))


class RngStream:
    POOL = (0, 1, 2, 3, 4)
    PNP_PLAN_SEL = 5
    PNP_PLAN_SUBSETS = 6
    PNP_SUBSETS = 7
    UMEYAMA_OWN = 8
    UMEYAMA_POSE = 9
    UMEYAMA_PLAN = 10


def device_seed(table: Dict[int, torch.Tensor], device) -> torch.Tensor:
    idx = device.index or 0
    if idx not in table:
        table[idx] = torch.zeros(1, dtype=torch.int64, device=device)
    return table[idx]


def conv_tile(M: int, N: int, K: int = 1024, nchw: bool = False) -> int:
    if nchw:
        return 6 if N <= 96 else 3
    if N <= 32:
        return 6
    return 8


TILE_SHAPES = {1: (128, 128, 16), 2: (128, 64, 16), 3: (64, 64, 16), 4: (128, 128, 32), 5: (256, 32, 16),
               6: (128, 32, 32), 7: (128, 64, 32), 8: (64, 64, 32)}


SPLITK = knobs.flag("KRRN_SPLITK")
SPLITK_TILES = 256
SPLITK_NKT = 8
SPLITK_PER = 4


def conv_splits(M: int, N: int, K: int, tile: int) -> int:
    BM, BN, BK = TILE_SHAPES[tile]
    cd = lambda a, b: (a + b - 1) // b
    tiles = cd(M, BM) * cd(N, BN)
    nkt = cd(K, BK)
    if tiles >= SPLITK_TILES or nkt < SPLITK_NKT or N % 4 or not SPLITK:
        return 1
    return max(1, min(cd(512, tiles), nkt // SPLITK_PER, 16))


CONV_KERNELS = {1: "conv_gemm_f32<128,128,16>", 2: "conv_gemm_f32<128,64,16>", 3: "conv_gemm_f32<64,64,16>",
                4: "conv_gemm_f32<128,128,32>", 5: "conv_gemm_f32<256,32,16>", 6: "conv_gemm_f32<128,32,32>",
                7: "conv_gemm_f32<128,64,32>", 8: "conv_gemm_f32<64,64,32>"}


_iarr = ops._int_array


X3_TILE = 2


def add_conv(plan: Plan, *, x, x_cs, x_co, B, Hi, Wi, cin_p, Hg, Wg, in_s, taps, wt, N, n_store, scale, bias,
             bias2=None, b2_div=1, res=None, res_cs=0, res_co=0, out, out_cs, out_co, Ho, Wo, osy=1, osx=1, ooy=0,
             oox=0, relu=False, nchw=False, cin=None, cout=None, tag="", tile=None, splits=None, wt3=None):
    M = B * Hg * Wg
    K = cin_p * len(taps)
    tile_req = tile
    tile = conv_tile(M, N, K, nchw) if tile is None else tile
    if splits is None:
        splits = 1 if nchw else conv_splits(M, N, K, tile)
    ws = plan.scratch(splits * M * N) if splits > 1 else None
    cin = cin_p if cin is None else cin
    cout = n_store if cout is None else cout
    flops = 2.0 * cin * cout * len(taps) * M
    kname = CONV_KERNELS[tile] + (",nchw" if nchw else "") + (",splitk" if splits > 1 else "")
    if wt3 is not None and not nchw and N > 32 and splits == 1:
        tile = X3_TILE if tile_req is None else tile_req
        kname = CONV_KERNELS[tile]
        plan.add("krrn_conv2d_x3_f32", x, x_cs, x_co, B, Hi, Wi, cin_p, Hg, Wg, in_s, len(taps),
                 _iarr([t[0] for t in taps]), _iarr([t[1] for t in taps]), wt3, N, n_store, scale, bias,
                 bias2 if bias2 is not None else P(0), b2_div, res if res is not None else P(0), res_cs, res_co, out,
                 out_cs, out_co, Ho, Wo, osy, osx, ooy, oox, int(relu), tile, splits, ptr(ws),
                 meta=dict(kernel=kname.replace("conv_gemm_f32", "conv_gemm_x3"), flops=flops, tag=tag, M=M, N=N,
                           K=K, splits=splits, mfma_flops=2.0 * M * N * K * 6 / 16,
                           mfma_bf16_flops=2.0 * M * N * K * 6))
        return
    plan.add("krrn_conv2d_f32", x, x_cs, x_co, B, Hi, Wi, cin_p, Hg, Wg, in_s, len(taps), _iarr([t[0] for t in taps]),
             _iarr([t[1] for t in taps]), wt, N, n_store, scale, bias, bias2 if bias2 is not None else P(0), b2_div,
             res if res is not None else P(0), res_cs, res_co, out, out_cs, out_co, Ho, Wo, osy, osx, ooy, oox,
             int(relu), int(nchw), tile, splits, ptr(ws),
             meta=dict(kernel=kname, flops=flops, tag=tag, M=M, N=N, K=K, splits=splits))


GROUP_TILE = 6


def conv_desc(*, x, x_cs, x_co, B, Hi, Wi, cin_p, Hg, Wg, in_s, taps, wt, N, n_store, scale, bias, res=None,
              res_cs=0, res_co=0, out, out_cs, out_co, Ho, Wo, osy=1, osx=1, ooy=0, oox=0, relu=False,
              splits=1, ws=None, k_chunk=0) -> ConvDesc:
    d = ConvDesc()
    d.in_, d.in_cs, d.in_co, d.B, d.Hi, d.Wi, d.cin, d.Hg, d.Wg, d.in_s = x, x_cs, x_co, B, Hi, Wi, cin_p, Hg, Wg, in_s
    d.ntaps = len(taps)
    for i, (dy, dx) in enumerate(taps):
        d.tap_dy[i], d.tap_dx[i] = dy, dx
    d.wt, d.N, d.n_store, d.scale, d.bias, d.bias2, d.b2_div = wt, N, n_store, scale, bias, P(0), 1
    d.res = res if res is not None else P(0)
    d.res_cs, d.res_co = res_cs, res_co
    d.out, d.out_cs, d.out_co, d.Ho, d.Wo = out, out_cs, out_co, Ho, Wo
    d.osy, d.osx, d.ooy, d.oox, d.relu, d.out_nchw = osy, osx, ooy, oox, int(relu), 0
    d.splits, d.workspace = splits, (ws if ws is not None else P(0))
    d.k_chunk = k_chunk
    return d


def add_conv_group(plan: Plan, problems: List[dict], tile: int = None, tag: str = "group", x3: bool = False):
    tile = GROUP_TILE if tile is None else tile
    n = len(problems)
    arr = (ConvDesc * n)()
    flops = 0.0
    nsplit = 1
    shapes = []
    for q, pr in enumerate(problems):
        pr = dict(pr)
        cin, cout = pr.pop("cin"), pr.pop("cout")
        M = pr["B"] * pr["Hg"] * pr["Wg"]
        K = pr["cin_p"] * len(pr["taps"])
        sp = conv_splits(M, pr["N"], K, tile)
        ws = ptr(plan.scratch(sp * M * pr["N"], slot=q)) if sp > 1 else None
        arr[q] = conv_desc(**pr, splits=sp, ws=ws)
        flops += 2.0 * cin * cout * len(pr["taps"]) * M
        nsplit = max(nsplit, sp)
        shapes.append((M, pr["N"], K, sp))
    plan.buffers.append(arr)
    meta = dict(kernel=f"conv_group{'_x3' if x3 else ''}<{','.join(map(str, TILE_SHAPES[tile]))}>", flops=flops,
                tag=tag, M=shapes[0][0], N=shapes[0][1], K=shapes[0][2], splits=nsplit, shapes=shapes)
    if x3:
        pipe = sum(2.0 * M * N * K for M, N, K, _ in shapes)
        meta.update(mfma_flops=pipe * 6 / 16, mfma_bf16_flops=pipe * 6)
    plan.add("krrn_conv2d_group_x3_f32" if x3 else "krrn_conv2d_group_f32", ctypes.cast(arr, P), n, tile, meta=meta)


BLAS = knobs.flag("KRRN_BLAS")
BLAS_MAX_WS = 64 << 20
GEMM_X3 = knobs.flag("KRRN_GEMM_X3")
GEMM_PANEL = knobs.flag("KRRN_GEMM_PANEL")
GEMM_X3_MINK = 256


class _BlasPlan:

    def __init__(self, handle):
        self.handle = handle

    def __del__(self):
        try:
            if self.handle:
                _lib.lib().krrn_blas_gemm_destroy(self.handle)
        except Exception:
            pass


def add_gemm(plan: Plan, *, a: torch.Tensor, a_off: int, lda: int, M: int, wt: torch.Tensor, K: int, N: int,
             scale: Optional[torch.Tensor], bias: Optional[torch.Tensor], out: torch.Tensor, ldo: int, relu: bool,
             res: Optional[torch.Tensor] = None, ldr: int = 0, batch: int = 1, a_grp: int = 0, o_grp: int = 0,
             r_grp: int = 0, cin: Optional[int] = None, cout: Optional[int] = None, tag: str = "gemm",
             require_x3: bool = False, blas_ok: bool = True) -> bool:
    dev = plan.device
    w = wt.reshape(N, -1)[:, :K].float()
    if scale is not None:
        w = w * scale.reshape(N, 1).to(w.device)
    w = w.contiguous()
    wkey = (wt.data_ptr(), scale.data_ptr() if scale is not None else 0, K, N)

    def packed(kind: str, fn):
        key = wkey + (kind,)
        if key not in plan._packed:
            plan._packed[key] = fn(w)
        plan.buffers.append([plan._packed[key], wt, scale, bias])
        return plan._packed[key]
    flops = 2.0 * (cin or K) * (cout or N) * M * batch
    if GEMM_PANEL and not require_x3 and K in (64, 128) and N % 32 == 0 and N <= 2048 and batch == 1 \
            and lda % 4 == 0 and a_off % 4 == 0 and not (K == 128 and res is not None):
        wp = packed("panel", ops.gemm_weights_panel)
        csplit = 1
        tiles = N // 32
        if K == 128:
            blocks = (M + 127) // 128
            while tiles % (2 * csplit) == 0 and (tiles // csplit > 16 or
                                                 (blocks * csplit < 512 and tiles // csplit >= 16)):
                csplit *= 2
        else:
            rows = (M + 255) // 256
            while rows * csplit < 256 and tiles % (2 * csplit) == 0:
                csplit *= 2
        plan.add("krrn_gemm_panel_x3_f32", P(a.data_ptr() + 4 * a_off), lda, M, K, N, ptr(wp), ptr(bias), ptr(res),
                 ldr, ptr(out), ldo, int(relu), csplit,
                 meta=dict(kernel="gemm_panel_x3", flops=flops, tag=tag, M=M, N=N, K=K, splits=csplit,
                           mfma_flops=2.0 * M * N * K * 6 / 16, mfma_bf16_flops=2.0 * M * N * K * 6,
                           bytes=4.0 * (M * K + M * N)))
        return True
    if GEMM_X3 and K >= GEMM_X3_MINK and K % 32 == 0 and N % 128 == 0 and lda % 4 == 0 and ldo % 4 == 0 and a_off % 4 == 0 \
            and (res is None or ldr % 4 == 0):
        w3 = packed("x3", ops.gemm_weights_x3)
        plan.add("krrn_gemm_x3_f32", P(a.data_ptr() + 4 * a_off), lda, M, K, N, ptr(w3), ptr(bias), ptr(res), ldr,
                 ptr(out), ldo, int(relu), batch, a_grp, o_grp, r_grp,
                 meta=dict(kernel="gemm_x3", flops=flops, tag=tag, M=M * batch, N=N, K=K, splits=1,
                           mfma_flops=2.0 * M * batch * N * K * 6 / 16, mfma_bf16_flops=2.0 * M * batch * N * K * 6))
        return True
    if not BLAS or require_x3 or not blas_ok:
        return False
    h = ctypes.c_void_p()
    wsb = ctypes.c_longlong()
    st = _lib.lib().krrn_blas_gemm_create(M, N, K, lda, ldo, batch, a_grp, o_grp, int(bias is not None), int(relu),
                                          int(res is not None), ldr, r_grp, BLAS_MAX_WS, ctypes.byref(h),
                                          ctypes.byref(wsb))
    if st != 0:
        return False
    owner = _BlasPlan(h)
    ws = plan.buf((max(int(wsb.value), 16),), torch.uint8, zero=False)
    plan.buffers.append([owner, w, bias])
    a_ptr = P(a.data_ptr() + 4 * a_off)
    plan.add("krrn_blas_gemm_run", h, a_ptr, ptr(w), ptr(bias), ptr(res), ptr(out), ptr(ws), int(wsb.value),
             meta=dict(kernel="hipblaslt_gemm_f32", flops=2.0 * (cin or K) * (cout or N) * M * batch, tag=tag,
                       M=M * batch, N=N, K=K, splits=1))
    return True
```

Measured before the change: 6247 crops/s.

## Compute TBase MLP only on distinct (nn1,nn2) pairs via pair compaction

Adds a pair-compaction kernel that deduplicates each sample's (nn1, nn2) nearest-neighbour index pairs into a compact list, a per-point slot map and a live count. The TBase conv2 and conv3 GEMMs then run only on the distinct rows, with tiles past the live count exiting early, and the tail scatters results back through the slot map. This cuts redundant MLP work when many points share the same coarse-level neighbours, at the cost of an extra compaction kernel with a large shared-memory bitmap. The fusion code also gains an early-geometry hook. Everything is gated behind the KRRN_TBASE_GATHER and KRRN_TBASE_DISTINCT flags.

```diff
diff --git a/include/krrn_hip.h b/include/krrn_hip.h
--- a/include/krrn_hip.h
+++ b/include/krrn_hip.h
@@ -67,6 +67,14 @@
                             long long a2_bs, int a2_st, int npts, int B, int K, int N, const void* w3f,
                             const float* bias, float* out, int ldo, int relu, void* stream);
 
+int krrn_gemm_x3_live_f32(const float* a, int lda, int M, int K, int N, const void* w3f, const float* bias,
+                          const float* res, int ldr, float* out, int ldo, int relu, int batch, long long a_grp,
+                          long long o_grp, long long r_grp, const int* live, void* stream);
+int krrn_gemm_x3_gather_live_f32(const int* ia, const float* A, long long a_bs, int a_st, const int* ib,
+                                 const float* A2, long long a2_bs, int a2_st, int npts, int B, int K, int N,
+                                 const void* w3f, const float* bias, float* out, int ldo, int relu, const int* live,
+                                 void* stream);
+
 int krrn_gemm_panel_x3_f32(const float* a, int lda, int M, int K, int N, const void* wpf, const float* bias,
                            const float* res, int ldr, float* out, int ldo, int relu, int csplit, void* stream);
 
@@ -139,6 +147,12 @@
 int krrn_tbase_tail_f32(const float* h, int B, int n, int C, const float* w4, const float* b4, const float* cloud,
                         float* pred_t, float* t_res, void* stream);
 
+int krrn_tbase_tail_slot_f32(const float* h, const int* slot, int B, int n, int C, const float* w4, const float* b4,
+                             const float* cloud, float* pred_t, float* t_res, void* stream);
+
+int krrn_pair_compact_i32(const int* ia, const int* ib, int B, int npts, int n1, int n2, int* cnt, int* pa, int* pb,
+                          int* slot, void* stream);
+
 int krrn_pnp_ransac_f32(const float* xyz, int HW, const long long* choose, int N, const int* sel, int P,
                         const float* xmap, const float* ymap, const float* K4, const double* extent,
                         const double* lfborder, const int* subsets, int H, float thr, double conf, float* workspace,
diff --git a/pose_estimation_amd/csrc/gemm_x3.hip b/pose_estimation_amd/csrc/gemm_x3.hip
--- a/pose_estimation_amd/csrc/gemm_x3.hip
+++ b/pose_estimation_amd/csrc/gemm_x3.hip
@@ -14,7 +14,8 @@
   const int* ia;
   const int* ib;
   long long a2_grp;
-  int lda2, npts;
+  int lda2, npts, nb, i_grp;
+  const int* live;
   const unsigned* w;
   const float* bias;
   const float* res;
@@ -40,6 +41,7 @@
   const int grp = bid / tpg, rem = bid - grp * tpg;
   const int tm = rem / g.nt, tn = rem - tm * g.nt;
   const int m0 = tm * BM, n0 = tn * BN;
+  if (g.live && m0 >= g.live[grp]) return;
   const int tid = threadIdx.x, lane = tid & 63, wave = tid >> 6;
   const int frow = lane & 31, fh = lane >> 5;
 
@@ -47,19 +49,20 @@
   const float* abase = GA ? g.a : g.a + grp * g.a_grp + (size_t)m0 * g.lda;
   const int rows = min(BM, g.M - m0);
   const __amdgpu_buffer_rsrc_t rsA = __builtin_amdgcn_make_buffer_rsrc(
-      (void*)abase, (short)0, GA ? (int)(g.a_grp * (g.M / g.npts) * 4) : ((rows - 1) * g.lda + g.K) * 4, 0x00020000);
+      (void*)abase, (short)0, GA ? (int)(g.a_grp * g.nb * 4) : ((rows - 1) * g.lda + g.K) * 4, 0x00020000);
   __amdgpu_buffer_rsrc_t rsA2;
   unsigned aoff[2], aoff2[2];
   if constexpr (GA) {
-    rsA2 = __builtin_amdgcn_make_buffer_rsrc((void*)g.a2, (short)0, (int)(g.a2_grp * (g.M / g.npts) * 4),
+    rsA2 = __builtin_amdgcn_make_buffer_rsrc((void*)g.a2, (short)0, (int)(g.a2_grp * g.nb * 4),
                                              0x00020000);
 #pragma unroll
     for (int i = 0; i < 2; ++i) {
       const int m = m0 + srow + 64 * i;
       if (m < g.M) {
-        const int b = m / g.npts;
-        aoff[i] = (unsigned)((b * g.a_grp + (long long)g.ia[m] * g.lda + kq) * 4);
-        aoff2[i] = (unsigned)((b * g.a2_grp + (long long)g.ib[m] * g.lda2 + kq) * 4);
+        const int b = g.i_grp ? grp : m / g.npts;
+        const long long ii = (long long)grp * g.i_grp + m;
+        aoff[i] = (unsigned)((b * g.a_grp + (long long)g.ia[ii] * g.lda + kq) * 4);
+        aoff2[i] = (unsigned)((b * g.a2_grp + (long long)g.ib[ii] * g.lda2 + kq) * 4);
       } else {
         aoff[i] = aoff2[i] = 0x80000000u;
       }
@@ -211,9 +214,11 @@
 
 }
 
-KRRN_API int krrn_gemm_x3_f32(const float* a, int lda, int M, int K, int N, const void* w3f, const float* bias,
-                              const float* res, int ldr, float* out, int ldo, int relu, int batch, long long a_grp,
-                              long long o_grp, long long r_grp, void* stream) {
+namespace {
+
+int launch_plain(const float* a, int lda, int M, int K, int N, const void* w3f, const float* bias, const float* res,
+                 int ldr, float* out, int ldo, int relu, int batch, long long a_grp, long long o_grp,
+                 long long r_grp, const int* live, void* stream) {
   if (!a || !w3f || !out) return KRRN_EARG;
   if (M < 1 || K < KC || N < BN || batch < 1) return KRRN_ESHAPE;
   if ((K % (2 * KC)) || (N % BN) || lda < K || ldo < N) return KRRN_ESHAPE;
@@ -224,7 +229,8 @@
   const long long tiles = (long long)krrn_cdiv(M, BM) * (N / BN) * batch;
   if (tiles > 0x7FFFFFFFLL) return KRRN_ESHAPE;
   GemmArgs g;
-  g.a = a; g.a2 = nullptr; g.ia = g.ib = nullptr; g.a2_grp = 0; g.lda2 = 0; g.npts = 1;
+  g.a = a; g.a2 = nullptr; g.ia = g.ib = nullptr; g.a2_grp = 0; g.lda2 = 0; g.npts = 1; g.nb = 1; g.i_grp = 0;
+  g.live = live;
   g.w = reinterpret_cast<const unsigned*>(w3f); g.bias = bias; g.res = res; g.out = out;
   g.lda = lda; g.M = M; g.K = K; g.N = N; g.ldr = ldr; g.ldo = ldo; g.relu = relu;
   g.a_grp = a_grp; g.o_grp = o_grp; g.r_grp = r_grp;
@@ -233,10 +239,9 @@
   return krrn_launch_status();
 }
 
-KRRN_API int krrn_gemm_x3_gather_f32(const int* ia, const float* A, long long a_bs, int a_st, const int* ib,
-                                     const float* A2, long long a2_bs, int a2_st, int npts, int B, int K, int N,
-                                     const void* w3f, const float* bias, float* out, int ldo, int relu,
-                                     void* stream) {
+int launch_gather(const int* ia, const float* A, long long a_bs, int a_st, const int* ib, const float* A2,
+                  long long a2_bs, int a2_st, int npts, int B, int K, int N, const void* w3f, const float* bias,
+                  float* out, int ldo, int relu, const int* live, void* stream) {
   if (!ia || !A || !ib || !A2 || !w3f || !out) return KRRN_EARG;
   if (npts < 1 || B < 1 || K < KC || N < BN) return KRRN_ESHAPE;
   if ((K % (2 * KC)) || (N % BN) || a_st < K || a2_st < K || ldo < N) return KRRN_ESHAPE;
@@ -244,15 +249,48 @@
   if (!krrn_aligned16(A) || !krrn_aligned16(A2) || !krrn_aligned16(w3f) || !krrn_aligned16(out)) return KRRN_EALIGN;
   if ((long long)B * a_bs * 4 >= 0x7FFFFFFFLL || (long long)B * a2_bs * 4 >= 0x7FFFFFFFLL) return KRRN_ESHAPE;
   const long long M = (long long)B * npts;
-  const long long tiles = (long long)krrn_cdiv(M, BM) * (N / BN);
+  const long long tiles = live ? (long long)krrn_cdiv(npts, BM) * (N / BN) * B : (long long)krrn_cdiv(M, BM) * (N / BN);
   if (M > 0x7FFFFFFFLL || tiles > 0x7FFFFFFFLL) return KRRN_ESHAPE;
   GemmArgs g;
   g.a = A; g.a2 = A2; g.ia = ia; g.ib = ib; g.a_grp = a_bs; g.a2_grp = a2_bs; g.lda = a_st; g.lda2 = a2_st;
-  g.npts = npts;
+  g.npts = npts; g.nb = B; g.i_grp = live ? npts : 0; g.live = live;
   g.w = reinterpret_cast<const unsigned*>(w3f); g.bias = bias; g.res = nullptr; g.out = out;
-  g.M = (int)M; g.K = K; g.N = N; g.ldr = 0; g.ldo = ldo; g.relu = relu;
-  g.o_grp = 0; g.r_grp = 0;
+  g.M = live ? npts : (int)M; g.K = K; g.N = N; g.ldr = 0; g.ldo = ldo; g.relu = relu;
+  g.o_grp = live ? (long long)npts * ldo : 0; g.r_grp = 0;
   g.mt = krrn_cdiv(g.M, BM); g.nt = N / BN; g.total = (int)tiles;
   hipLaunchKernelGGL(gemm_x3_kernel<true>, dim3((unsigned)tiles), dim3(256), 0, (hipStream_t)stream, g);
   return krrn_launch_status();
 }
+
+}
+
+KRRN_API int krrn_gemm_x3_f32(const float* a, int lda, int M, int K, int N, const void* w3f, const float* bias,
+                              const float* res, int ldr, float* out, int ldo, int relu, int batch, long long a_grp,
+                              long long o_grp, long long r_grp, void* stream) {
+  return launch_plain(a, lda, M, K, N, w3f, bias, res, ldr, out, ldo, relu, batch, a_grp, o_grp, r_grp, nullptr,
+                      stream);
+}
+
+KRRN_API int krrn_gemm_x3_live_f32(const float* a, int lda, int M, int K, int N, const void* w3f, const float* bias,
+                                   const float* res, int ldr, float* out, int ldo, int relu, int batch,
+                                   long long a_grp, long long o_grp, long long r_grp, const int* live, void* stream) {
+  if (!live) return KRRN_EARG;
+  return launch_plain(a, lda, M, K, N, w3f, bias, res, ldr, out, ldo, relu, batch, a_grp, o_grp, r_grp, live, stream);
+}
+
+KRRN_API int krrn_gemm_x3_gather_f32(const int* ia, const float* A, long long a_bs, int a_st, const int* ib,
+                                     const float* A2, long long a2_bs, int a2_st, int npts, int B, int K, int N,
+                                     const void* w3f, const float* bias, float* out, int ldo, int relu,
+                                     void* stream) {
+  return launch_gather(ia, A, a_bs, a_st, ib, A2, a2_bs, a2_st, npts, B, K, N, w3f, bias, out, ldo, relu, nullptr,
+                       stream);
+}
+
+KRRN_API int krrn_gemm_x3_gather_live_f32(const int* ia, const float* A, long long a_bs, int a_st, const int* ib,
+                                          const float* A2, long long a2_bs, int a2_st, int npts, int B, int K, int N,
+                                          const void* w3f, const float* bias, float* out, int ldo, int relu,
+                                          const int* live, void* stream) {
+  if (!live) return KRRN_EARG;
+  return launch_gather(ia, A, a_bs, a_st, ib, A2, a2_bs, a2_st, npts, B, K, N, w3f, bias, out, ldo, relu, live,
+                       stream);
+}
diff --git a/pose_estimation_amd/csrc/pointwise.hip b/pose_estimation_amd/csrc/pointwise.hip
--- a/pose_estimation_amd/csrc/pointwise.hip
+++ b/pose_estimation_amd/csrc/pointwise.hip
@@ -192,6 +192,7 @@
                                                          const float* __restrict__ w4,
                                                          const float* __restrict__ b4,
                                                          const float* __restrict__ cloud,
+                                                         const int* __restrict__ slot,
                                                          float* __restrict__ pred_t, float* __restrict__ t_res) {
   __shared__ float red[kTailWaves][3];
   const int b = blockIdx.x;
@@ -203,7 +204,8 @@
   for (int i0 = 0; i0 < n; i0 += 16 * kTailWaves) {
     const int i = i0 + wave * 16 + pl;
     if (i < n) {
-      const f32x4* hr = reinterpret_cast<const f32x4*>(h + ((long long)b * n + i) * C);
+      const int r = slot ? slot[(long long)b * n + i] : i;
+      const f32x4* hr = reinterpret_cast<const f32x4*>(h + ((long long)b * n + r) * C);
       float a0 = 0.f, a1 = 0.f, a2 = 0.f;
       for (int c4 = q; c4 < C4; c4 += 4) {
         const f32x4 x = hr[c4];
@@ -275,6 +277,73 @@
   *reinterpret_cast<f32x4*>(out + b * o_bs + (long long)i * o_st + 4 * c4) = v;
 }
 
+__device__ __forceinline__ int pair_key(int a, int b, int n1, int n2) {
+  return min(max(a, 0), n1 - 1) * n2 + min(max(b, 0), n2 - 1);
+}
+constexpr int kPairThreads = 256;
+constexpr int kPairWords = 8192;
+__global__ __launch_bounds__(kPairThreads) void pair_compact_kernel(const int* __restrict__ ia,
+                                                                    const int* __restrict__ ib, int npts, int n1,
+                                                                    int n2, int words, int* __restrict__ cnt,
+                                                                    int* __restrict__ pa, int* __restrict__ pb,
+                                                                    int* __restrict__ slot) {
+  __shared__ unsigned bits[kPairWords];
+  __shared__ unsigned short pre[kPairWords];
+  __shared__ int part[kPairThreads];
+  __shared__ int first_key;
+  const int b = blockIdx.x, tid = threadIdx.x;
+  const int* ka = ia + (long long)b * npts;
+  const int* kb = ib + (long long)b * npts;
+  for (int w = tid; w < words; w += kPairThreads) bits[w] = 0u;
+  __syncthreads();
+  for (int i = tid; i < npts; i += kPairThreads) {
+    const int key = pair_key(ka[i], kb[i], n1, n2);
+    atomicOr(&bits[key >> 5], 1u << (key & 31));
+  }
+  __syncthreads();
+  const int per = (words + kPairThreads - 1) / kPairThreads;
+  const int w0 = min(tid * per, words), w1 = min(w0 + per, words);
+  int mine = 0;
+  for (int w = w0; w < w1; ++w) mine += __popc(bits[w]);
+  part[tid] = mine;
+  __syncthreads();
+  for (int off = 1; off < kPairThreads; off <<= 1) {
+    const int v = tid >= off ? part[tid - off] : 0;
+    __syncthreads();
+    part[tid] += v;
+    __syncthreads();
+  }
+  const int total = part[kPairThreads - 1];
+  int rank = part[tid] - mine;
+  int* qa = pa + (long long)b * npts;
+  int* qb = pb + (long long)b * npts;
+  for (int w = w0; w < w1; ++w) {
+    pre[w] = (unsigned short)rank;
+    unsigned m = bits[w];
+    while (m) {
+      const int key = 32 * w + __ffs(m) - 1;
+      m &= m - 1;
+      if (rank == 0) first_key = key;
+      qa[rank] = key / n2;
+      qb[rank] = key - (key / n2) * n2;
+      ++rank;
+    }
+  }
+  __syncthreads();
+  if (tid == 0) cnt[b] = total;
+  const int a0 = first_key / n2, b0 = first_key - a0 * n2;
+  for (int j = total + tid; j < npts; j += kPairThreads) {
+    qa[j] = a0;
+    qb[j] = b0;
+  }
+  int* sl = slot + (long long)b * npts;
+  for (int i = tid; i < npts; i += kPairThreads) {
+    const int key = pair_key(ka[i], kb[i], n1, n2);
+    const int w = key >> 5;
+    sl[i] = (int)pre[w] + __popc(bits[w] & ((1u << (key & 31)) - 1u));
+  }
+}
+
 inline dim3 grid1(long long total) { return dim3((unsigned)((total + 255) / 256)); }
 
 }
@@ -391,8 +460,29 @@
   if (!h || !w4 || !b4 || !cloud || !pred_t) return KRRN_EARG;
   if (B < 1 || n < 1 || C < 1) return KRRN_ESHAPE;
   if ((C & 3) || !krrn_aligned16(h) || !krrn_aligned16(w4)) return KRRN_EALIGN;
-  hipLaunchKernelGGL(tbase_tail_kernel, dim3(B), dim3(64 * kTailWaves), 0, (hipStream_t)stream, h, n, C, w4, b4, cloud, pred_t,
-                     t_res);
+  hipLaunchKernelGGL(tbase_tail_kernel, dim3(B), dim3(64 * kTailWaves), 0, (hipStream_t)stream, h, n, C, w4, b4, cloud,
+                     (const int*)nullptr, pred_t, t_res);
+  return krrn_launch_status();
+}
+
+KRRN_API int krrn_tbase_tail_slot_f32(const float* h, const int* slot, int B, int n, int C, const float* w4,
+                                      const float* b4, const float* cloud, float* pred_t, float* t_res,
+                                      void* stream) {
+  if (!h || !slot || !w4 || !b4 || !cloud || !pred_t) return KRRN_EARG;
+  if (B < 1 || n < 1 || C < 1) return KRRN_ESHAPE;
+  if ((C & 3) || !krrn_aligned16(h) || !krrn_aligned16(w4)) return KRRN_EALIGN;
+  hipLaunchKernelGGL(tbase_tail_kernel, dim3(B), dim3(64 * kTailWaves), 0, (hipStream_t)stream, h, n, C, w4, b4, cloud,
+                     slot, pred_t, t_res);
+  return krrn_launch_status();
+}
+
+KRRN_API int krrn_pair_compact_i32(const int* ia, const int* ib, int B, int npts, int n1, int n2, int* cnt, int* pa,
+                                   int* pb, int* slot, void* stream) {
+  if (!ia || !ib || !cnt || !pa || !pb || !slot) return KRRN_EARG;
+  if (B < 1 || npts < 1 || n1 < 1 || n2 < 1) return KRRN_ESHAPE;
+  if ((long long)n1 * n2 > 32LL * kPairWords || npts > 0xFFFF) return KRRN_ESHAPE;
+  hipLaunchKernelGGL(pair_compact_kernel, dim3(B), dim3(kPairThreads), 0, (hipStream_t)stream, ia, ib, npts, n1, n2,
+                     (n1 * n2 + 31) / 32, cnt, pa, pb, slot);
   return krrn_launch_status();
 }
 
diff --git a/pose_estimation_amd/fusion.py b/pose_estimation_amd/fusion.py
--- a/pose_estimation_amd/fusion.py
+++ b/pose_estimation_amd/fusion.py
@@ -69,6 +69,8 @@
 
 FEAT_SID = 4
 FUSION_CHUNK = knobs.integer("KRRN_FUSION_CHUNK")
+GEOM_EARLY = knobs.flag("KRRN_GEOM_EARLY")
+GEOM_SID = 8
 
 def level_sizes(N: int, k0: int):
     N1 = int(N / 4)
@@ -195,25 +197,78 @@
     e = _Emit(fu, plan, B, keep)
     knn, gcn, gemm, off = e.knn, e.gcn, e.gemm, _off
 
+    def pool_knn(bi, br):
+        knn(off(p9, 3 * bi), N * 9, 9, N1, ptr(perms[br]), off(p9, 3 * bi), N * 9, 9, N, 3, 4, 1, 0, nb4[br])
+
+    def pool_verts(bi, br):
+        plan.add("krrn_gather_rows_f32", ptr(perms[br]), 0, 0, N1, off(p9, 3 * bi), N * 9, 9, off(V1, 3 * bi),
+                 N1 * 9, 9, 3, B)
+
+    def pool1_verts():
+        plan.add("krrn_gather_rows_f32", ptr(perms["p1"]), 0, 0, N1, off(p9, 0), N * 9, 9, off(PV1, 0), N1 * 9, 9, 9, B)
+
+    def knn_idx1():
+        knn(off(V1, 0), N1 * 9, 9, N1, ptr(None), off(V1, 0), N1 * 9, 9, N1, 3, k1, 1, 0, idx1)
+
+    def knn_nn1():
+        knn(off(p9, 0), N * 9, 9, N, ptr(None), off(PV1, 0), N1 * 9, 9, N1, 3, 1, 0, 1, nn1)
+
+    def pool2_knn():
+        knn(off(PV1, 0), N1 * 9, 9, N2, ptr(perms["p2"]), off(PV1, 0), N1 * 9, 9, N1, 3, 4, 1, 0, nb4b)
+
+    def pool2_verts():
+        plan.add("krrn_gather_rows_f32", ptr(perms["p2"]), 0, 0, N2, off(PV1, 0), N1 * 9, 9, off(PV2, 0), N2 * 9, 9, 9, B)
+
+    def knn_idx2():
+        knn(off(PV2, 0), N2 * 9, 9, N2, ptr(None), off(PV2, 0), N2 * 9, 9, N2, 9, k2, 1, 0, idx2)
+
+    def knn_nn2():
+        knn(off(p9, 0), N * 9, 9, N, ptr(None), off(PV2, 0), N2 * 9, 9, N2, 3, 1, 0, 1, nn2)
+
+    geom = GEOM_EARLY
+
+    def on_geom(*fns):
+        with plan.on_stream(GEOM_SID):
+            for fn in fns:
+                fn()
+
+    def wait_geom(dst):
+        if dst == 0:
+            plan.sync(GEOM_SID, 0)
+        else:
+            plan.edge(GEOM_SID, dst)
+
     if not early:
         knn(off(p9, 0), N * 9, 9, N, ptr(None), off(p9, 0), N * 9, 9, N, 3, k0, 1, 0, idx0)
+    if geom:
+        plan.fork([GEOM_SID])
+        on_geom(*[lambda bi=bi, br=br: pool_knn(bi, br) for bi, br in enumerate(("v", "x", "n"))],
+                *[lambda bi=bi, br=br: pool_verts(bi, br) for bi, br in enumerate(("v", "x", "n"))], pool1_verts)
     plan.fork([1, 2])
     for bi, br in enumerate(("v", "x", "n")):
         with plan.on_stream(bi):
             if not (early and bi == 0):
                 _level0_branch(e, fu, bi, br, N, idx0, off(p9, 3 * bi), N * 9, 9, F0, Y1[bi], feat1, cy)
-            perm = perms[br]
-            knn(off(p9, 3 * bi), N * 9, 9, N1, ptr(perm), off(p9, 3 * bi), N * 9, 9, N, 3, 4, 1, 0, nb4[br])
+            if geom:
+                wait_geom(bi)
+            else:
+                pool_knn(bi, br)
             plan.add("krrn_pool_max_f32", ptr(nb4[br]), N1, 4, off(feat1, 128 * bi), N * 384, 384, 128,
                      off(FP1, 128 * bi), N1 * 384, 384, B)
-            plan.add("krrn_gather_rows_f32", ptr(perm), 0, 0, N1, off(p9, 3 * bi), N * 9, 9, off(V1, 3 * bi),
-                     N1 * 9, 9, 3, B)
-    plan.add("krrn_gather_rows_f32", ptr(perms["p1"]), 0, 0, N1, off(p9, 0), N * 9, 9, off(PV1, 0), N1 * 9, 9, 9, B)
+            if not geom:
+                pool_verts(bi, br)
+    if not geom:
+        pool1_verts()
     plan.join([1, 2])
-    knn(off(V1, 0), N1 * 9, 9, N1, ptr(None), off(V1, 0), N1 * 9, 9, N1, 3, k1, 1, 0, idx1)
-    plan.fork([1, 2, 3])
-    with plan.on_stream(3):
-        knn(off(p9, 0), N * 9, 9, N, ptr(None), off(PV1, 0), N1 * 9, 9, N1, 3, 1, 0, 1, nn1)
+    if geom:
+        on_geom(knn_idx1)
+        wait_geom(0)
+        plan.fork([1, 2])
+    else:
+        knn_idx1()
+        plan.fork([1, 2, 3])
+        with plan.on_stream(3):
+            knn_nn1()
     for bi, br in enumerate(("v", "x", "n")):
         with plan.on_stream(bi):
             c2 = getattr(fu, f"conv_2_{br}")
@@ -223,22 +278,36 @@
     plan.join([1, 2])
     for h in hooks.get("level1", []):
         h(dict(feat1=feat1, feat2=feat2))
-    knn(off(PV1, 0), N1 * 9, 9, N2, ptr(perms["p2"]), off(PV1, 0), N1 * 9, 9, N1, 3, 4, 1, 0, nb4b)
+    if geom:
+        on_geom(pool2_knn, pool2_verts, knn_idx2)
+        wait_geom(0)
+    else:
+        pool2_knn()
     plan.add("krrn_pool_max_f32", ptr(nb4b), N2, 4, off(feat2, 0), N1 * 384, 384, 384, off(FP2, 0), N2 * 384, 384, B)
-    plan.add("krrn_gather_rows_f32", ptr(perms["p2"]), 0, 0, N2, off(PV1, 0), N1 * 9, 9, off(PV2, 0), N2 * 9, 9, 9, B)
-    knn(off(PV2, 0), N2 * 9, 9, N2, ptr(None), off(PV2, 0), N2 * 9, 9, N2, 9, k2, 1, 0, idx2)
+    if not geom:
+        pool2_verts()
+        knn_idx2()
     for h in hooks.get("level2", []):
         h(dict(feat1=feat1, feat2=feat2))
-    plan.fork([3])
-    with plan.on_stream(3):
-        knn(off(p9, 0), N * 9, 9, N, ptr(None), off(PV2, 0), N2 * 9, 9, N2, 3, 1, 0, 1, nn2)
+    pair_hooks = [lambda h=h: h(dict(nn1=nn1, nn2=nn2)) for h in hooks.get("pairs", [])]
+    if geom:
+        on_geom(knn_nn1, knn_nn2, *pair_hooks)
+    else:
+        plan.fork([3])
+        with plan.on_stream(3):
+            knn_nn2()
+            for h in pair_hooks:
+                h()
     gemm(FP2, 384, 0, B * N2, fu.conv_4, Y4)
     gcn(idx2, N2, k2, off(PV2, 0), N2 * 9, 9, _dn(fu.conv_4.directions, dev), 512, Y4, None, False,
         off(fm4, 0), N2 * 512, 512)
     gemm(fm4, 512, 0, B * N2, fu.conv_5, Y5)
     gcn(idx2, N2, k2, off(PV2, 0), N2 * 9, 9, _dn(fu.conv_5.directions, dev), 512, Y5, None, False,
         off(fm5, 0), N2 * 512, 512)
-    plan.join([3])
+    if geom:
+        wait_geom(0)
+    else:
+        plan.join([3])
     if materialize:
         plan.fork([FEAT_SID])
         with plan.on_stream(FEAT_SID):
diff --git a/pose_estimation_amd/knobs.py b/pose_estimation_amd/knobs.py
--- a/pose_estimation_amd/knobs.py
+++ b/pose_estimation_amd/knobs.py
@@ -36,6 +36,12 @@
     "KRRN_TBASE_EARLY": ("1", "TBase conv1's level-1 half runs as soon as level 1 is done (side stream)"),
     "KRRN_TBASE_GATHER": ("1", "TBase conv1 / conv2 by linearity on the fusion's level rows (gathered "
                                "GEMM); 0 = on the materialised 1280-wide concat"),
+    "KRRN_TBASE_DISTINCT": ("1", "with KRRN_TBASE_GATHER, TBase conv2 / conv3 run once per distinct (nn1, nn2) "
+                                 "pair of a crop and the tail reads each point's row by its slot (same bits); "
+                                 "0 = once per point"),
+    "KRRN_GEOM_EARLY": ("0", "1 = the fusion launches that read only p9 and the perms (pool kNNs, vertex gathers, "
+                             "idx1, idx2, nn1, nn2) run on their own plan stream from the level-0 kNN on "
+                             "(same bits; measured 0.6 % slower); 0 = where their consumers are"),
     "KRRN_POSE_AT": ("level1", "where the fused pose step forks off the forward plan: level1 / level2 / heads"),
     "KRRN_FUSION_CHUNK": ("16", "crops per chunk of the level-0 GCN GEMM + gather-conv, through a chunk-sized "
                                 "Y buffer per branch (0 = the whole batch at once; same results)"),
diff --git a/pose_estimation_amd/krrn.py b/pose_estimation_amd/krrn.py
--- a/pose_estimation_amd/krrn.py
+++ b/pose_estimation_amd/krrn.py
@@ -13,7 +13,7 @@
 from .fusion import FEAT_SID, FusionNetLite, build_fusion_plan, emit_fusion_cloud_part, level_sizes
 from .hrnet import _Builder, build_hrnet, build_hrnet_plan
 from .ops import Act, pad4
-from .posenet import PoseNet, build_tbase_plan, emit_tbase_level1
+from .posenet import PoseNet, build_tbase_plan, emit_pair_compact, emit_tbase_level1
 from .runtime import Late, Plan, RngStream, add_conv, h2d, ptr
 
 
@@ -136,6 +136,9 @@
 
             if TBASE_EARLY:
                 hooks["level1"].append(tracked(emit_tb_l1))
+            tb_pairs = {}
+            hooks["pairs"] = [tracked(lambda fb: tb_pairs.update(
+                emit_pair_compact(plan, B, N, N1, N2, fb["nn1"], fb["nn2"]) or {}))]
             f0 = len(plan.ops)
             feat, self.fusion_bufs = build_fusion_plan(model.fusion, plan, B, N, self.p9, self.perms, hooks=hooks,
                                                        materialize=model.keep_fusion_feat, early=early)
@@ -147,7 +150,8 @@
                           N2=N2)
             self.pred_t, self.tbase_bufs = build_tbase_plan(model.pose.t_net, plan, B, N, feat, "cls", "cloud",
                                                             cfg.Module.POSENet.INC_R, C, levels=levels,
-                                                            pre=tb_pre or None, pre_sid=tb_sid)
+                                                            pre=tb_pre or None, pre_sid=tb_sid,
+                                                            pairs=tb_pairs or None)
             if feat is not None:
                 plan.join([FEAT_SID])
         if pose_hook is not None:
diff --git a/pose_estimation_amd/posenet.py b/pose_estimation_amd/posenet.py
--- a/pose_estimation_amd/posenet.py
+++ b/pose_estimation_amd/posenet.py
@@ -10,6 +10,8 @@
 
 
 TBASE_GATHER = knobs.flag("KRRN_TBASE_GATHER")
+TBASE_DISTINCT = knobs.flag("KRRN_TBASE_DISTINCT")
+PAIR_MAX_KEYS = 1 << 18
 
 
 class TBase(nn.Module):
@@ -88,8 +90,20 @@
     return dict(P1=P1, Q=Q)
 
 
+def emit_pair_compact(plan: Plan, B: int, N: int, N1: int, N2: int, nn1: torch.Tensor,
+                      nn2: torch.Tensor) -> Optional[dict]:
+    if not (TBASE_GATHER and TBASE_DISTINCT) or N1 * N2 > PAIR_MAX_KEYS or N > 0xFFFF:
+        return None
+    i32 = torch.int32
+    pr = dict(cnt=plan.buf((B,), i32), pa=plan.buf((B, N), i32), pb=plan.buf((B, N), i32), slot=plan.buf((B, N), i32))
+    plan.add("krrn_pair_compact_i32", ptr(nn1), ptr(nn2), B, N, N1, N2, ptr(pr["cnt"]), ptr(pr["pa"]), ptr(pr["pb"]),
+             ptr(pr["slot"]))
+    return pr
+
+
 def build_tbase_plan(tb: TBase, plan: Plan, B: int, N: int, feat: torch.Tensor, cls_key: str, cloud_key: str,
-                     inc_r: int, num_cls: int, levels=None, pre: Optional[dict] = None, pre_sid: int = 0):
+                     inc_r: int, num_cls: int, levels=None, pre: Optional[dict] = None, pre_sid: int = 0,
+                     pairs: Optional[dict] = None):
     dev = plan.device
     w1, spec1, colv = _conv1_fold(tb, inc_r, num_cls, dev)
     np1 = ops.pad4(1024)
@@ -98,6 +112,10 @@
     w4 = tb.conv4.weight.detach()[:3, :, 0].float().contiguous().to(dev)
     b4 = tb.conv4.bias.detach()[:3].float().contiguous().to(dev)
     gathered = levels is not None and TBASE_GATHER
+    if gathered and pairs is None:
+        pairs = emit_pair_compact(plan, B, N, levels["N1"], levels["N2"], levels["nn1"], levels["nn2"])
+    if not gathered:
+        pairs = None
     h1 = None if gathered else plan.buf((B * N, 1024))
     h2 = plan.buf((B * N, 256))
     h3 = plan.buf((B * N, 256))
@@ -143,18 +161,32 @@
             w2 = tb.conv2.weight.detach()[:, :, 0].to(dev).float() * spec2.scale[:256].reshape(256, 1)
             w3 = ops.gemm_weights_x3(w2.contiguous())
             keep += [w3]
-            plan.add("krrn_gemm_x3_gather_f32", ptr(levels["nn1"]), ptr(P1), N1 * np1, np1, ptr(levels["nn2"]),
-                     ptr(P2), N2 * np1, np1, N, B, 1024, 256, ptr(w3), ptr(spec2.bias), ptr(h2), 256, 1,
-                     meta=dict(kernel="gemm_x3", flops=2.0 * 1024 * 256 * M, tag="tbase_gemm", M=M, N=256, K=1024,
-                               splits=1, mfma_flops=2.0 * M * 256 * 1024 * 6 / 16,
-                               mfma_bf16_flops=2.0 * M * 256 * 1024 * 6))
+            meta = dict(kernel="gemm_x3", flops=2.0 * 1024 * 256 * M, tag="tbase_gemm", M=M, N=256, K=1024,
+                        splits=1, mfma_flops=2.0 * M * 256 * 1024 * 6 / 16, mfma_bf16_flops=2.0 * M * 256 * 1024 * 6)
+            if pairs is not None:
+                plan.add("krrn_gemm_x3_gather_live_f32", ptr(pairs["pa"]), ptr(P1), N1 * np1, np1, ptr(pairs["pb"]),
+                         ptr(P2), N2 * np1, np1, N, B, 1024, 256, ptr(w3), ptr(spec2.bias), ptr(h2), 256, 1,
+                         ptr(pairs["cnt"]), meta=meta)
+            else:
+                plan.add("krrn_gemm_x3_gather_f32", ptr(levels["nn1"]), ptr(P1), N1 * np1, np1, ptr(levels["nn2"]),
+                         ptr(P2), N2 * np1, np1, N, B, 1024, 256, ptr(w3), ptr(spec2.bias), ptr(h2), 256, 1,
+                         meta=meta)
         else:
             plan.add("krrn_gather2_add_f32", ptr(levels["nn2"]), ptr(P2), N2 * np1, np1, ptr(levels["nn1"]),
                      ptr(P1), N1 * np1, np1, N, np1, ptr(spec1.scale), ptr(spec1.bias), ptr(b2), 1, ptr(h1),
                      N * 1024, 1024, B)
     if not gathered:
         gemm(h1, 1024, spec2, h2)
-    gemm(h2, 256, spec3, h3)
-    plan.add("krrn_tbase_tail_f32", ptr(h3), B, N, 256, ptr(w4), ptr(b4), Late(cloud_key), ptr(pred_t), ptr(None))
+    if pairs is not None:
+        if not add_gemm(plan, a=h2, a_off=0, lda=256, M=N, wt=spec3.wt[0], K=spec3.cin_p, N=ops.pad4(spec3.cout),
+                        scale=spec3.scale, bias=spec3.bias, out=h3, ldo=256, relu=True, batch=B, a_grp=N * 256,
+                        o_grp=N * 256, cin=spec3.cin, cout=spec3.cout, tag="tbase_gemm", require_x3=True,
+                        live=pairs["cnt"]):
+            raise RuntimeError("TBase on distinct rows needs the split-bf16 GEMM (KRRN_GEMM_X3=1)")
+        plan.add("krrn_tbase_tail_slot_f32", ptr(h3), ptr(pairs["slot"]), B, N, 256, ptr(w4), ptr(b4),
+                 Late(cloud_key), ptr(pred_t), ptr(None))
+    else:
+        gemm(h2, 256, spec3, h3)
+        plan.add("krrn_tbase_tail_f32", ptr(h3), B, N, 256, ptr(w4), ptr(b4), Late(cloud_key), ptr(pred_t), ptr(None))
     plan.buffers.append(keep)
-    return pred_t, dict(h1=h1, h2=h2, h3=h3)
+    return pred_t, dict(h1=h1, h2=h2, h3=h3, **(pairs or {}))
diff --git a/pose_estimation_amd/runtime.py b/pose_estimation_amd/runtime.py
--- a/pose_estimation_amd/runtime.py
+++ b/pose_estimation_amd/runtime.py
@@ -395,7 +395,7 @@
              scale: Optional[torch.Tensor], bias: Optional[torch.Tensor], out: torch.Tensor, ldo: int, relu: bool,
              res: Optional[torch.Tensor] = None, ldr: int = 0, batch: int = 1, a_grp: int = 0, o_grp: int = 0,
              r_grp: int = 0, cin: Optional[int] = None, cout: Optional[int] = None, tag: str = "gemm",
-             require_x3: bool = False, blas_ok: bool = True) -> bool:
+             require_x3: bool = False, blas_ok: bool = True, live: Optional[torch.Tensor] = None) -> bool:
     dev = plan.device
     w = wt.reshape(N, -1)[:, :K].float()
     if scale is not None:
@@ -410,6 +410,8 @@
         plan.buffers.append([plan._packed[key], wt, scale, bias])
         return plan._packed[key]
     flops = 2.0 * (cin or K) * (cout or N) * M * batch
+    if live is not None and not require_x3:
+        raise ValueError("a live-row GEMM runs on gemm_x3 only (require_x3=True)")
     if GEMM_PANEL and not require_x3 and K in (64, 128) and N % 32 == 0 and N <= 2048 and batch == 1 \
             and lda % 4 == 0 and a_off % 4 == 0 and not (K == 128 and res is not None):
         wp = packed("panel", ops.gemm_weights_panel)
@@ -433,8 +435,9 @@
     if GEMM_X3 and K >= GEMM_X3_MINK and K % 32 == 0 and N % 128 == 0 and lda % 4 == 0 and ldo % 4 == 0 and a_off % 4 == 0 \
             and (res is None or ldr % 4 == 0):
         w3 = packed("x3", ops.gemm_weights_x3)
-        plan.add("krrn_gemm_x3_f32", P(a.data_ptr() + 4 * a_off), lda, M, K, N, ptr(w3), ptr(bias), ptr(res), ldr,
-                 ptr(out), ldo, int(relu), batch, a_grp, o_grp, r_grp,
+        tail = () if live is None else (ptr(live),)
+        plan.add("krrn_gemm_x3_f32" if live is None else "krrn_gemm_x3_live_f32", P(a.data_ptr() + 4 * a_off), lda, M,
+                 K, N, ptr(w3), ptr(bias), ptr(res), ldr, ptr(out), ldo, int(relu), batch, a_grp, o_grp, r_grp, *tail,
                  meta=dict(kernel="gemm_x3", flops=flops, tag=tag, M=M * batch, N=N, K=K, splits=1,
                            mfma_flops=2.0 * M * batch * N * K * 6 / 16, mfma_bf16_flops=2.0 * M * batch * N * K * 6))
         return True
```

Result: faster. 6315 crops/s (median of 6 runs) (+1.1%).
